# MartinErhardt/RoaringRegex

Measured on AMD Instinct MI355X. Metric: GB/s input scanned (whole job), 256-state regex, higher is better.
Workload: dtype u32

## Files before the change

### roaringregex_amd/csrc/corpus.cpp

```cpp
#include <algorithm>
#include <cstring>

#include "handles.hpp"

using namespace rrx;

namespace {
constexpr int kMailSlots = 64, kMailWords = 8;
struct MailPage { uint64_t *host = nullptr, *dev = nullptr; std::vector<int> free_slots; };
std::mutex g_mail_mu;
std::map<int, MailPage> g_mail;
}
int mailbox_acquire(int device, Mailbox *out) {
    std::lock_guard<std::mutex> lock(g_mail_mu);
    MailPage &pg = g_mail[device];
    if (!pg.host) {
        PinnedAlloc h;
        void *d = nullptr;
        hipError_t e = h.alloc(kMailSlots * kMailWords * sizeof(uint64_t), hipHostMallocMapped);
        if (e == hipSuccess) e = hipHostGetDevicePointer(&d, h.p, 0);
        if (e != hipSuccess) return hip_fail(e, "hipHostMalloc(mailbox)");
        pg.host = static_cast<uint64_t *>(h.release()); pg.dev = static_cast<uint64_t *>(d);
        for (int i = kMailSlots - 1; i >= 0; i--) pg.free_slots.push_back(i);
    }
    if (pg.free_slots.empty()) return fail(RRX_ERR_HIP, "more than 64 synchronous calls in flight on one device");
    out->slot = pg.free_slots.back(); pg.free_slots.pop_back();
    out->device = device;
    out->host = pg.host + (size_t)out->slot * kMailWords;
    out->dev = pg.dev + (size_t)out->slot * kMailWords;
    return RRX_OK;
}
void mailbox_release(const Mailbox &m) {
    if (m.slot < 0) return;
    std::lock_guard<std::mutex> lock(g_mail_mu);
    g_mail[m.device].free_slots.push_back(m.slot);
}

static constexpr uint32_t kSampleGroups = 8, kSampleBytes = 256;
static constexpr size_t kSampleMinCorpus = (size_t)64 << 20;

extern "C" {

int rrx_corpus_create(int device, const void *d_bytes, size_t nbytes, void *stream, rrx_corpus **out) {
    return rrx_corpus_create_ex(device, d_bytes, nbytes, 0, stream, out);
}

int rrx_corpus_create_ex(int device, const void *d_bytes, size_t nbytes, uint32_t stripe_bytes, void *stream, rrx_corpus **out) {
    if (!out || (nbytes && !d_bytes)) return fail(RRX_ERR_ARG, "null argument");
    if (stripe_bytes && (stripe_bytes < dev::kMinStripe || stripe_bytes > dev::kMaxStripe || (stripe_bytes & (stripe_bytes - 1))))
        return fail(RRX_ERR_ARG, "stripe must be a power of two in [512, 16384]");
    if (reinterpret_cast<uintptr_t>(d_bytes) & 15) return fail(RRX_ERR_ARG, "corpus base must be 16-byte aligned");
    *out = nullptr;
    HIP_TRY(hipSetDevice(device));
    std::unique_ptr<rrx_corpus> c(new rrx_corpus());
    c->device = device;
    c->d_bytes = static_cast<const uint8_t *>(d_bytes);
    c->nbytes = nbytes;
    c->stripe = stripe_bytes ? stripe_bytes : dev::pick_stripe(nbytes);
    constexpr size_t kSample = (size_t)4 << 20;
    if (!stripe_bytes && nbytes >= 16 * kSample) {
        rrx_corpus *sample = nullptr;
        if (rrx_corpus_create_ex(device, d_bytes, kSample, dev::pick_stripe(kSample), stream, &sample) == RRX_OK && sample) {
            if (sample->nlines) c->stripe = dev::stripe_for_lines(nbytes, kSample / sample->nlines);
            rrx_corpus_free(sample);
        }
    }
    c->nstripes = (nbytes + c->stripe - 1) / c->stripe;
    hipError_t e = c->d_counts.alloc(device, (c->nstripes + 3) * sizeof(uint32_t));
    if (e == hipSuccess) e = c->d_base.alloc(device, (c->nstripes + 1 + dev::scan_scratch_words(c->nstripes)) * sizeof(uint64_t));
    if (e != hipSuccess) return hip_fail(e, "hipMalloc(line index)");
    uint32_t *d_flags = c->d_counts + c->nstripes;
    e = hipMemsetAsync(d_flags, 0, 3 * sizeof(uint32_t), (hipStream_t)stream);
    if (e != hipSuccess) return hip_fail(e, "hipMemsetAsync(flags)");
    int rc = dev::count_newlines_per_stripe(c->d_bytes, nbytes, c->stripe, c->d_counts, c->nstripes, d_flags, stream);
    if (!rc) rc = dev::scan_counts(c->d_counts, c->d_base, c->d_base + c->nstripes + 1, c->nstripes, stream);
    if (!rc && c->nstripes) rc = dev::own_words_check(c->d_base, c->nstripes, c->d_bytes + nbytes - 1, d_flags + 1, stream);
    if (rc) return hip_fail((hipError_t)rc, "line index launch");
    MailboxGuard mail;
    if (int mrc = mailbox_acquire(device, &mail.m)) return mrc;
    if (nbytes >= kSampleMinCorpus && c->nstripes >= 64 * kSampleGroups &&
        c->h_sample.alloc((size_t)kSampleGroups * 32 * kSampleBytes) == hipSuccess) {
        c->sample_lanes = kSampleGroups * 32;
        for (uint32_t g = 0; g < kSampleGroups; g++) {
            const size_t first_stripe = (size_t)g * (c->nstripes / kSampleGroups);
            if (hipMemcpy2DAsync(c->h_sample + (size_t)g * 32 * kSampleBytes, kSampleBytes, c->d_bytes + first_stripe * c->stripe, c->stripe,
                                 kSampleBytes, 32, hipMemcpyDeviceToHost, (hipStream_t)stream) != hipSuccess) {
                (void)hipGetLastError();
                (void)hipStreamSynchronize((hipStream_t)stream);
                c->h_sample.reset(); c->sample_lanes = 0;
                break;
            }
        }
    }
    mail.stream = (hipStream_t)stream; mail.queued = true;
    rc = dev::mail_results(c->d_base + c->nstripes, d_flags, nbytes ? c->d_bytes + nbytes - 1 : nullptr, mail.m.dev, stream, d_flags + 1);
    if (rc) return hip_fail((hipError_t)rc, "line index launch");
    e = hipStreamSynchronize((hipStream_t)stream);
    if (e != hipSuccess) return hip_fail(e, "line index readback");
    mail.drained = true;
    const uint64_t total = mail.m.host[0];
    const uint32_t flags = (uint32_t)mail.m.host[1];
    const uint8_t last = nbytes ? (uint8_t)mail.m.host[2] : (uint8_t)'\n';
    c->has_high = (flags & 1u) != 0;
    c->own_words = c->nstripes && mail.m.host[3] == 0;
    c->own_span = (uint32_t)mail.m.host[4];
    c->nlines = (size_t)total + ((nbytes && last != '\n') ? 1 : 0);
    if (!stripe_bytes && c->nlines) {
        const uint32_t want = dev::stripe_for_lines(nbytes, nbytes / c->nlines);
        if (want != c->stripe) {
            c.reset();
            return rrx_corpus_create_ex(device, d_bytes, nbytes, want, stream, out);
        }
    }
    *out = c.release();
    return RRX_OK;
}
size_t rrx_corpus_num_lines(const rrx_corpus *c) { return c->nlines; }
size_t rrx_corpus_num_bytes(const rrx_corpus *c) { return c->nbytes; }
uint32_t rrx_corpus_stripe_bytes(const rrx_corpus *c) { return c->stripe; }
int rrx_corpus_one_launch(const rrx_corpus *c, uint32_t *span_words) {
    if (span_words) *span_words = c->own_words ? c->own_span : 0;
    return c->own_words ? 1 : 0;
}
void rrx_corpus_free(rrx_corpus *c) { delete c; }

size_t rrx_corpus_bitmap_words(const rrx_corpus *c) { return (c->nlines + 31) / 32; }

static int match_corpus_sampled(const rrx_regex *re, const rrx_corpus *c, const DeviceTables *t, uint32_t *d_accept_bits, void *stream) {
    dev::Dfa2Device d2;
    int rc = re->sampled_tables(c->device, &d2);
    if (rc) return rc;
    hipStream_t st = (hipStream_t)stream;
    const size_t words = rrx_corpus_bitmap_words(c);
    const size_t wide_bytes = (2 * words * sizeof(uint32_t) + 15) & ~(size_t)15, esc_bytes = (words * sizeof(uint32_t) + 15) & ~(size_t)15;
    const size_t cap = std::max<size_t>(words / 2, 1024);
    std::lock_guard<std::mutex> lock(re->onepass_mu);
    void *buf = nullptr;
    rc = re->onepass_for(c->device, wide_bytes + esc_bytes + cap * sizeof(uint64_t), &buf, st);
    if (rc) return rc;
    uint32_t *wide = static_cast<uint32_t *>(buf);
    uint32_t *escaped = reinterpret_cast<uint32_t *>(static_cast<uint8_t *>(buf) + wide_bytes);
    uint64_t *list = reinterpret_cast<uint64_t *>(static_cast<uint8_t *>(buf) + wide_bytes + esc_bytes);
    DeviceAlloc &count = re->sampled_dev.escapes[c->device];
    if (!count.p) HIP_TRY(count.alloc(c->device, 16));
    unsigned long long *total = static_cast<unsigned long long *>(count.p);
    constexpr uint32_t kSlots = kSampledRelearns + 1;
    PinnedArray<unsigned long long> &all_seen = re->sampled_dev.seen;
    if (!all_seen && all_seen.alloc(kSlots * sizeof(unsigned long long)) == hipSuccess)
        for (uint32_t k = 0; k < kSlots; k++) all_seen[k] = 0;
    unsigned long long *const seen = all_seen ? all_seen + re->sampled.seen_slot() : nullptr;
    if (seen) re->sampled.judge(seen[0]);
    hipError_t he = hipMemsetAsync(wide, 0, wide_bytes, st);
    if (he == hipSuccess) he = hipMemsetAsync(total, 0, 16, st);
    int e = he != hipSuccess ? (int)he : dev::match_stripes_dfa2_two_bit(d2, c->d_bytes, c->nbytes, c->stripe, c->d_base, c->nstripes, wide, stream);
    if (!e) e = dev::split_two_bit(wide, c->nlines, d_accept_bits, escaped, total, list, cap, stream);
    if (!e) e = dev::recheck_escaped_nfa(t->nfa, c->d_bytes, c->nbytes, c->stripe, c->d_base, c->nstripes, escaped, c->nlines, list, total, cap, d_accept_bits, stream);
    if (!e && seen) {
        if (hipMemcpyAsync(seen, total, sizeof(unsigned long long), hipMemcpyDeviceToHost, st) != hipSuccess) (void)hipGetLastError();
        re->sampled.queued(c->nlines);
    }
    const int rc2 = re->onepass_done(c->device, st);
    if (e) return hip_fail((hipError_t)e, "sampled-table launch");
    return rc2;
}

static unsigned long long *own_words_for(const rrx_corpus *c, const dev::Dfa2Device &d2, hipStream_t stream) {
    if (!c->own_words || c->own_span >= dev::dfa2_window_words(d2)) return nullptr;
    hipStreamCaptureStatus capture = hipStreamCaptureStatusNone;
    if (hipStreamIsCapturing(stream, &capture) != hipSuccess) { (void)hipGetLastError(); return nullptr; }
    if (capture != hipStreamCaptureStatusNone) return nullptr;
    std::lock_guard<std::mutex> lock(c->mu);
    auto it = c->slot_arrays.find(stream);
    if (it != c->slot_arrays.end()) return it->second;
    if (c->slot_arrays.size() >= rrx_corpus::kMaxSlotArrays) return nullptr;
    const size_t bytes = ((c->nstripes + dev::kThreads - 1) / dev::kThreads + 1) * sizeof(unsigned long long);
    DeviceArray<unsigned long long> slots;
    if (slots.alloc(c->device, bytes) != hipSuccess || hipMemsetAsync(slots, 0, bytes, stream) != hipSuccess) { (void)hipGetLastError(); return nullptr; }
    return c->slot_arrays.emplace(stream, std::move(slots)).first->second;
}
static uint32_t flush_mask_of(const rrx_regex *re, const rrx_corpus *c) {
    return re->opt_flush_slots.load() ? (uint32_t)re->opt_flush_slots.load() - 1u : dev::flush_mask_for(c->nbytes, c->nlines);
}
uint32_t rrx_match_flush_slots(const rrx_regex *re, const rrx_corpus *c, int *compiled_in) {
    const uint32_t mask = flush_mask_of(re, c);
    if (compiled_in) *compiled_in = dev::dfa2_flush_at_compile_time(mask) ? 1 : 0;
    return mask + 1;
}

static int launch_line_tables(const rrx_regex *re, const rrx_corpus *c, const LineTables &lt, const DeviceTables *t, bool stride2_over_high, uint32_t *bits,
                              void *stream) {
    const size_t words = rrx_corpus_bitmap_words(c);
    const bool stride2 = lt.has_dfa2 && (!c->has_high || stride2_over_high);
    dev::Dfa2Device d2;
    unsigned long long *slots = nullptr;
    if (stride2) { d2 = re->dfa2_device(t); slots = own_words_for(c, d2, (hipStream_t)stream); }
    if (!slots) HIP_TRY(hipMemsetAsync(bits, 0, words * sizeof(uint32_t), (hipStream_t)stream));
    if (!stride2) return launched(dev::match_stripes_dfa(t->line, c->has_high, c->d_bytes, c->nbytes, c->stripe, c->d_base, c->nstripes, bits, stream), "match_stripes launch");
    return launched(dev::match_stripes_dfa2(d2, c->has_high, c->d_bytes, c->nbytes, c->stripe, c->d_base, c->nstripes, bits, stream, flush_mask_of(re, c), slots, words),
                    "match_stripes launch");
}

int rrx_match_corpus(const rrx_regex *re, const rrx_corpus *c, uint32_t *d_accept_bits, void *stream) {
    if (!re || !c || (c->nlines && !d_accept_bits)) return fail(RRX_ERR_ARG, "null argument");
    if (!re->t2_order.decided() && c->h_sample && !c->has_high) (void)re->decide_t2_order(c->h_sample, c->sample_lanes, kSampleBytes, false);
    const DeviceTables *t;
    int rc = re->tables(c->device, &t);
    if (rc) return rc;
    HIP_TRY(hipSetDevice(c->device));
    if (!c->nlines) return RRX_OK;
    const bool sampled_on = re->opt_sampled_table.load() != 0;
    if (re->sampled.eligible() && sampled_on && !c->has_high) {
        const bool beside = re->opt_background_order.load() != 0;
        if (c->h_sample) (void)re->sampled.start_first(c->h_sample, c->sample_lanes, kSampleBytes, beside);
        if (c->h_sample && re->sampled.ready() && re->sampled.retired())
            re->sampled.start_relearn(c->h_sample, c->sample_lanes, kSampleBytes, beside);
        if (re->sampled.in_use(sampled_on)) return match_corpus_sampled(re, c, t, d_accept_bits, stream);
    }
    if (re->engine == RRX_ENGINE_DFA)
        return launch_line_tables(re, c, re->match, t, false, d_accept_bits, stream);
    HIP_TRY(hipMemsetAsync(d_accept_bits, 0, rrx_corpus_bitmap_words(c) * sizeof(uint32_t), (hipStream_t)stream));
    int e = 0;
    switch (re->engine) {
    case RRX_ENGINE_NFA_SPARSE: e = dev::match_stripes_sparse_nfa(t->block, c->d_bytes, c->nbytes, c->stripe, c->d_base, c->nstripes, d_accept_bits, stream); break;
    case RRX_ENGINE_NFA_BLOCK: e = dev::match_stripes_wave_nfa(t->block, c->d_bytes, c->nbytes, c->stripe, c->d_base, c->nstripes, d_accept_bits, stream); break;
    case RRX_ENGINE_NFA_WAVE: e = dev::match_stripes_group_nfa(t->group, c->d_bytes, c->nbytes, c->stripe, c->d_base, c->nstripes, d_accept_bits, stream); break;
    default: e = dev::match_stripes_nfa(t->nfa, c->d_bytes, c->nbytes, c->stripe, c->d_base, c->nstripes, d_accept_bits, stream);
    }
    return launched(e, "match_stripes launch");
}

int rrx_contains_corpus(const rrx_regex *re, const rrx_corpus *c, uint32_t *d_bits, void *stream) {
    if (!re || !c || (c->nlines && !d_bits)) return fail(RRX_ERR_ARG, "null argument");
    bool on_nfa = false, fill = false;
    const dev::NfaDevice *nfa = nullptr;
    int rc = re->contains_nfa_tables(c->device, &on_nfa, &nfa, &fill);
    if (rc) return rc;
    if (on_nfa) {
        HIP_TRY(hipSetDevice(c->device));
        if (!c->nlines) return RRX_OK;
        rc = fill_bitmap(d_bits, c->nlines, fill, stream);
        if (rc || !nfa) return rc;
        return launched(dev::contains_stripes_nfa(*nfa, c->d_bytes, c->nbytes, c->stripe, c->d_base, c->nstripes, d_bits, stream), "contains_stripes launch");
    }
    const DeviceTables *t;
    rc = re->contains_tables(c->device, &t);
    if (rc) return rc;
    HIP_TRY(hipSetDevice(c->device));
    if (!c->nlines) return RRX_OK;
    return launch_line_tables(re, c, re->contains_set.lt, t, true, d_bits, stream);
}
int rrx_bitmap_count(int device, const uint32_t *d_bits, size_t nlines, uint64_t *d_count, void *stream) {
    if (!d_count || (nlines && !d_bits)) return fail(RRX_ERR_ARG, "null argument");
    HIP_TRY(hipSetDevice(device));
    static_assert(sizeof(unsigned long long) == sizeof(uint64_t), "64-bit atomics");
    return launched(dev::bitmap_count(d_bits, nlines, reinterpret_cast<unsigned long long *>(d_count), stream), "bitmap_count launch");
}

int rrx_match_device(const rrx_regex *re, int device, const void *d_bytes, size_t nbytes, uint32_t *d_accept_bits, size_t cap_words,
                     size_t *nlines, void *stream) {
    if (!re || (nbytes && !d_bytes) || !nlines || (cap_words && !d_accept_bits)) return fail(RRX_ERR_ARG, "null argument");
    if (reinterpret_cast<uintptr_t>(d_bytes) & 15) return fail(RRX_ERR_ARG, "corpus base must be 16-byte aligned");
    *nlines = 0;
    HIP_TRY(hipSetDevice(device));
    if (!nbytes) return RRX_OK;
    hipStream_t st = static_cast<hipStream_t>(stream);
    const bool sampled = re->sampled.in_use(re->opt_sampled_table.load() != 0);
    if ((re->engine != RRX_ENGINE_DFA && re->engine != RRX_ENGINE_NFA) || sampled) {
        rrx_corpus *c = nullptr;
        int rc = rrx_corpus_create(device, d_bytes, nbytes, stream, &c);
        if (rc) return rc;
        *nlines = c->nlines;
        if (rrx_corpus_bitmap_words(c) > cap_words) rc = fail(RRX_ERR_ARG, "accept bitmap too small for the number of strings");
        if (!rc) rc = rrx_match_corpus(re, c, d_accept_bits, stream);
        const hipError_t e = hipStreamSynchronize(st);
        if (!rc && e != hipSuccess) rc = hip_fail(e, "match_device");
        rrx_corpus_free(c);
        return rc;
    }
    const DeviceTables *t;
    int rc = re->tables(device, &t);
    if (rc) return rc;
    const uint8_t *bytes = static_cast<const uint8_t *>(d_bytes);
    const uint32_t stripe = dev::pick_stripe(nbytes);
    const size_t nstripes = (nbytes + stripe - 1) / stripe;
    const size_t counts_bytes = ((nstripes + 2) * sizeof(uint32_t) + 15) & ~(size_t)15;
    const size_t base_bytes = (nstripes + 1 + dev::scan_scratch_words(nstripes)) * sizeof(uint64_t);
    const size_t slab_bytes = dev::onepass_slab_words(nstripes, stripe) * sizeof(uint32_t);
    std::lock_guard<std::mutex> lock(re->onepass_mu);
    void *buf = nullptr;
    rc = re->onepass_for(device, counts_bytes + base_bytes + slab_bytes, &buf, st);
    if (rc) return rc;
    uint32_t *d_counts = static_cast<uint32_t *>(buf);
    uint64_t *d_base = reinterpret_cast<uint64_t *>(static_cast<uint8_t *>(buf) + counts_bytes);
    uint32_t *d_slabs = reinterpret_cast<uint32_t *>(static_cast<uint8_t *>(buf) + counts_bytes + base_bytes);
    MailboxGuard mail;
    rc = mailbox_acquire(device, &mail.m);
    if (rc) return rc;
    if (cap_words) HIP_TRY(hipMemsetAsync(d_accept_bits, 0, cap_words * sizeof(uint32_t), st));
    int e = re->engine == RRX_ENGINE_NFA ? dev::match_onepass_nfa(t->nfa, bytes, nbytes, stripe, nstripes, d_counts, d_slabs, stream)
            : re->match.has_dfa2         ? dev::match_onepass_dfa2(re->dfa2_device(t), bytes, nbytes, stripe, nstripes, d_counts, d_slabs, stream)
                                         : dev::match_onepass_dfa(t->line, bytes, nbytes, stripe, nstripes, d_counts, d_slabs, stream);
    if (!e) e = dev::scan_counts(d_counts, d_base, d_base + nstripes + 1, nstripes, stream);
    if (!e) e = dev::compact_streams(d_counts, d_base, nstripes, stripe, d_slabs, d_accept_bits, cap_words, stream);
    mail.stream = st; mail.queued = true;
    if (!e) e = dev::mail_results(d_base + nstripes, nullptr, bytes + nbytes - 1, mail.m.dev, stream);
    if (e) return hip_fail((hipError_t)e, "one-pass launch");
    const hipError_t he = hipStreamSynchronize(st);
    if (he != hipSuccess) return hip_fail(he, "one-pass readback");
    mail.drained = true;
    *nlines = (size_t)mail.m.host[0] + ((uint8_t)mail.m.host[2] != '\n' ? 1 : 0);
    if ((*nlines + 31) / 32 > cap_words) return fail(RRX_ERR_ARG, "accept bitmap too small for the number of strings");
    return RRX_OK;
}

int rrx_bitmap_to_bytes(int device, const uint32_t *d_bits, size_t nlines, uint8_t *d_accept, void *stream) {
    if (nlines && (!d_bits || !d_accept)) return fail(RRX_ERR_ARG, "null argument");
    if (reinterpret_cast<uintptr_t>(d_accept) & 15) return fail(RRX_ERR_ARG, "byte buffer must be 16-byte aligned");
    HIP_TRY(hipSetDevice(device));
    return launched(dev::expand_bits(d_bits, nlines, d_accept, stream), "expand_bits launch");
}

static int match_host_chunk(const rrx_regex *re, int device, uint8_t *d_text, size_t len, hipStream_t st, uint32_t *d_bits,
                            uint8_t *d_acc, uint8_t *accept, size_t cap, size_t line_off, size_t *nlines_out) {
    rrx_corpus *c = nullptr;
    int rc = rrx_corpus_create(device, d_text, len, st, &c);
    if (rc) return rc;
    const size_t n = c->nlines;
    rc = rrx_match_corpus(re, c, d_bits, st);
    if (!rc) rc = rrx_bitmap_to_bytes(device, d_bits, n, d_acc, st);
    if (!rc && line_off < cap) {
        const size_t take = n < cap - line_off ? n : cap - line_off;
        hipError_t e = hipMemcpyAsync(accept + line_off, d_acc, take, hipMemcpyDeviceToHost, st);
        if (e != hipSuccess) rc = hip_fail(e, "accept readback");
    }
    hipError_t e = hipStreamSynchronize(st);
    if (!rc && e != hipSuccess) rc = hip_fail(e, "chunk sync");
    rrx_corpus_free(c);
    *nlines_out = n;
    return rc;
}

int rrx_match_host(const rrx_regex *re, int device, const void *bytes, size_t nbytes, uint8_t *accept, size_t cap, size_t *nlines) {
    if (!re || (nbytes && !bytes) || !nlines) return fail(RRX_ERR_ARG, "null argument");
    HIP_TRY(hipSetDevice(device));
    *nlines = 0;
    if (!nbytes) return RRX_OK;
    const uint8_t *host = static_cast<const uint8_t *>(bytes);
    const size_t kChunk = (size_t)256 << 20;
    const size_t buf_bytes = (nbytes < kChunk ? nbytes : kChunk) + 64;
    const size_t max_lines = buf_bytes;
    struct Lane {
        DeviceArray<uint8_t> text, acc;
        DeviceArray<uint32_t> bits;
        hipStream_t st = nullptr;
        ~Lane() { if (st) { (void)hipStreamSynchronize(st); (void)hipStreamDestroy(st); } }
    } lane[2];
    const int nbuf = nbytes > kChunk ? 2 : 1;
    int rc = RRX_OK;
    hipError_t e = hipSuccess;
    for (int i = 0; i < nbuf && e == hipSuccess; i++) {
        e = lane[i].text.alloc(device, buf_bytes);
        if (e == hipSuccess) e = lane[i].acc.alloc(device, max_lines + 64);
        if (e == hipSuccess) e = lane[i].bits.alloc(device, (max_lines / 32 + 4) * sizeof(uint32_t));
        if (e == hipSuccess) e = hipStreamCreate(&lane[i].st);
    }
    if (e != hipSuccess) rc = hip_fail(e, "pipeline buffers");

    std::vector<size_t> cuts{0};
    while (!rc && cuts.back() < nbytes) {
        size_t lo = cuts.back(), hi = lo + kChunk < nbytes ? lo + kChunk : nbytes;
        if (hi < nbytes) {
            size_t q = hi;
            while (q > lo && host[q - 1] != '\n') q--;
            if (q == lo) { rc = fail(RRX_ERR_UNSUPPORTED, "a single line longer than 256 MiB: use rrx_corpus_create on a device buffer"); break; }
            hi = q;
        }
        cuts.push_back(hi);
    }
    const size_t nchunks = cuts.size() - 1;
    size_t line_off = 0;
    if (!rc) {
        e = hipMemcpyAsync(lane[0].text, host, cuts[1] - cuts[0], hipMemcpyHostToDevice, lane[0].st);
        if (e != hipSuccess) rc = hip_fail(e, "chunk upload");
    }
    for (size_t i = 0; i < nchunks && !rc; i++) {
        const int cur = (int)(i & 1) % nbuf, nxt = (int)((i + 1) & 1) % nbuf;
        if (i + 1 < nchunks) {
            e = hipMemcpyAsync(lane[nxt].text, host + cuts[i + 1], cuts[i + 2] - cuts[i + 1], hipMemcpyHostToDevice, lane[nxt].st);
            if (e != hipSuccess) { rc = hip_fail(e, "chunk upload"); break; }
        }
        size_t n = 0;
        rc = match_host_chunk(re, device, lane[cur].text, cuts[i + 1] - cuts[i], lane[cur].st, lane[cur].bits, lane[cur].acc, accept, cap, line_off, &n);
        line_off += n;
    }
    for (int i = 0; i < nbuf; i++) if (lane[i].st) (void)hipStreamSynchronize(lane[i].st);
    *nlines = line_off;
    return rc;
}

}
```

### roaringregex_amd/csrc/device.hpp

```cpp
#pragma once
#include <cstddef>
#include <cstdint>

namespace rrx {
namespace dev {

#ifndef RRX_THREADS
#define RRX_THREADS 1024
#endif
constexpr int kThreads = RRX_THREADS;
constexpr uint32_t kMinStripe = 512, kMaxStripe = 16384, kMinAutoStripe = 2048;
constexpr size_t kTargetLanes = (size_t)1 << 21;
inline uint32_t pick_stripe(size_t nbytes) {
    uint32_t s = kMinStripe;
    while (s < kMinAutoStripe && nbytes / s > ((size_t)1 << 18)) s *= 2;
    while (s < kMaxStripe && nbytes / s > kTargetLanes) s *= 2;
    return s;
}
inline uint32_t stripe_for_lines(size_t nbytes, size_t avg_line) {
    uint32_t want = pick_stripe(nbytes);
    while (want < kMaxStripe && avg_line * 16 > want && nbytes / (2 * (size_t)want) >= ((size_t)1 << 18)) want *= 2;
    while (want > 1024 && (avg_line + 1) * 128 < want) want /= 2;
    return want;
}
constexpr int kRound = 128;
constexpr int kMaxNfaWords = 16;
constexpr uint32_t kWideColumns = 129;
constexpr uint32_t kWideMaxStates = 127;
constexpr uint32_t kClassedMaxEntries = 16384;

struct NfaMasks {
    uint32_t init[kMaxNfaWords], fin[kMaxNfaWords], chain[kMaxNfaWords], self[kMaxNfaWords], excm[kMaxNfaWords];
    uint32_t cgrp[kMaxNfaWords], ctgt[kMaxNfaWords];
};

struct NfaDevice {
    uint32_t W = 0, nbits = 0, any_exc = 0, any_carry = 0, any_self = 0;
    NfaMasks masks;
    const uint32_t *B = nullptr;
    const uint32_t *X = nullptr;
};

constexpr uint32_t kGroupMaxBits = 8192;
struct GroupNfaDevice {
    uint32_t G = 0, K = 0, nbits = 0, n_exc = 0, ncls = 0;
    uint32_t exc_mode = 0;
    uint32_t self_slots = 0;
    uint32_t b_slots = 0;
    uint32_t exc_slots = 0;
    const uint32_t *masks = nullptr;
    const uint32_t *Bcls = nullptr;
    const uint8_t *cls = nullptr;
    const uint16_t *xidx = nullptr;
    const uint32_t *X = nullptr;
};
inline bool group_geometry(uint32_t nbits, uint32_t *G, uint32_t *K) {
    static const uint32_t forms[][2] = {{8, 3}, {8, 4}, {16, 3}, {16, 4}, {32, 3}, {32, 4}, {32, 5}, {32, 8}};
    for (const auto &f : forms)
        if (nbits <= f[0] * f[1] * 32u) { *G = f[0]; *K = f[1]; return true; }
    return false;
}

constexpr uint32_t kBlockMaxBits = 65536;
struct WaveNfaDevice {
    uint32_t WL = 0, nbits = 0;
    uint32_t self_words = 0, exc_words = 0;
    const uint32_t *masks = nullptr;
    const uint32_t *Bbyte = nullptr;
    const uint32_t *xoff = nullptr;
    const uint32_t *xtgt = nullptr;
    uint32_t ncls = 0;
    const uint32_t *Bcls = nullptr;
    const uint8_t *cls = nullptr;
};

struct DfaDevice {
    uint32_t nstates = 0, ncls = 0, start = 0;
    const uint8_t *cls = nullptr;
    const uint16_t *next = nullptr;
    const uint8_t *acc = nullptr;
};

constexpr size_t kPlainDfaLdsBudget = 64 * 1024;

struct LineDfaDevice {
    uint32_t nrows = 0;
    uint32_t stride = 0;
    uint32_t start_off = 0;
    uint32_t wide = 0;
    uint32_t rep_log2 = 0;
    uint32_t in_global = 0;
    const uint32_t *table = nullptr;
    const uint8_t *cls = nullptr;
};

struct Dfa2Device {
    uint32_t nrows = 0, stride = 0, start_off = 0, rep_log2 = 0;
    const uint16_t *P = nullptr;
    const uint32_t *T2 = nullptr;
    const uint8_t *P8 = nullptr;
};
constexpr uint32_t kDfa2PStride = 130;
constexpr uint32_t kDfa2PBytes = 128 * kDfa2PStride * 2;
constexpr uint32_t kDfa2P8Stride = 136;
constexpr uint32_t kDfa2P8Bytes = 128 * kDfa2P8Stride;
constexpr uint32_t kDfa2PItemsBytes = (129 * kDfa2PStride * 2 + 15) & ~15u;
constexpr uint32_t kDfa2RegionBytes = 46 * 1024;
constexpr uint32_t kDfa2MaxTable = kDfa2RegionBytes - 4 * 1024;
constexpr uint32_t kDfa2TableBudget = 30 * 1024;


int match_stripes_dfa(const LineDfaDevice &p, bool clamp_high, const uint8_t *bytes, size_t nbytes, uint32_t stripe,
                      const uint64_t *stripe_base, size_t nstripes, uint32_t *accept_bits, void *stream);
uint32_t flush_mask_for(size_t nbytes, size_t nlines);
int match_stripes_dfa2(const Dfa2Device &p, bool clean, const uint8_t *bytes, size_t nbytes, uint32_t stripe, const uint64_t *stripe_base,
                       size_t nstripes, uint32_t *accept, void *stream, uint32_t flush_mask = 31u, unsigned long long *slots = nullptr,
                       size_t nwords = 0);
uint32_t dfa2_window_words(const Dfa2Device &p);
bool dfa2_flush_at_compile_time(uint32_t flush_mask);
int match_stripes_dfa2_two_bit(const Dfa2Device &p, const uint8_t *bytes, size_t nbytes, uint32_t stripe, const uint64_t *stripe_base,
                               size_t nstripes, uint32_t *wide_bits, void *stream);
int split_two_bit(const uint32_t *wide, size_t nlines, uint32_t *accept_bits, uint32_t *escaped_bits, unsigned long long *escaped_total, uint64_t *list,
                  size_t cap, void *stream);

size_t onepass_slab_words(size_t nstripes, uint32_t stripe);
int match_onepass_dfa2(const Dfa2Device &p, const uint8_t *bytes, size_t nbytes, uint32_t stripe, size_t nstripes, uint32_t *counts,
                       uint32_t *slabs, void *stream);
int match_onepass_dfa(const LineDfaDevice &p, const uint8_t *bytes, size_t nbytes, uint32_t stripe, size_t nstripes, uint32_t *counts,
                      uint32_t *slabs, void *stream);
int compact_streams(const uint32_t *counts, const uint64_t *stripe_base, size_t nstripes, uint32_t stripe, const uint32_t *slabs,
                    uint32_t *accept_bits, size_t cap_words, void *stream);
int match_extents_dfa(const DfaDevice &p, const uint8_t *bytes, const uint64_t *off, size_t nitems, uint32_t trim,
                      uint8_t *accept, void *stream, const uint32_t *only_if = nullptr);

int count_newlines_per_stripe(const uint8_t *bytes, size_t nbytes, uint32_t stripe, uint32_t *counts, size_t nstripes, uint32_t *flags, void *stream);
int scan_counts(const uint32_t *counts, uint64_t *base, uint64_t *chunk_sums, size_t n, void *stream);
size_t scan_scratch_words(size_t n);
int expand_bits(const uint32_t *bits, size_t nlines, uint8_t *out, void *stream);
int bitmap_count(const uint32_t *bits, size_t nlines, unsigned long long *count, void *stream);
int mail_results(const uint64_t *total, const uint32_t *flags, const uint8_t *last_byte, uint64_t *mail, void *stream, const uint32_t *own = nullptr);
int own_words_check(const uint64_t *stripe_base, size_t nstripes, const uint8_t *last_byte, uint32_t *own, void *stream);
int build_line_offsets(const uint8_t *bytes, size_t nbytes, uint32_t stripe, const uint64_t *stripe_base, size_t nstripes,
                       uint64_t *line_off, void *stream);
int empty_matches(const uint64_t *line_off, size_t nlines, uint32_t *count, const uint64_t *first, uint32_t *match_start, uint32_t *match_end,
                  void *stream, size_t cap = ~(size_t)0);

constexpr uint32_t kItemColumns = 131, kItemEndColumn = 129;
size_t items_index_bytes(size_t nbytes, size_t nitems);
size_t items_result_bytes(size_t nitems);
int items_index_build(size_t nbytes, const uint64_t *off, size_t nitems, uint32_t trim, void *index, uint32_t **flag, void *stream,
                      const uint8_t *resolve_base = nullptr, size_t min_bytes = 0);
struct ItemVerdicts {
    uint8_t *bytes = nullptr;
    uint32_t *bits = nullptr;
    ItemVerdicts(uint8_t *b) : bytes(b) {}
    ItemVerdicts(uint32_t *w) : bits(w) {}
};
int items_match2(const Dfa2Device &p, const uint8_t *bytes, size_t nbytes, size_t nitems, const void *index, void *result, ItemVerdicts out, void *stream,
                 const uint64_t *resolve_off = nullptr, const uint32_t *skip_if = nullptr);
int items_match(const LineDfaDevice &p, const uint8_t *bytes, size_t nbytes, size_t nitems, uint32_t trim, const void *index, void *result,
                ItemVerdicts out, void *stream, const uint64_t *resolve_off = nullptr, const uint32_t *skip_if = nullptr);

int contains_extents_dfa(const DfaDevice &p, bool in_global, uint32_t found, const uint8_t *bytes, const uint64_t *off, size_t nitems, uint32_t trim,
                         uint32_t *bits, void *stream, const uint32_t *only_if = nullptr);
int copy_result_bits(const uint32_t *result, size_t nitems, uint32_t *bits, void *stream);

struct MultiDevice {
    uint32_t nstates = 0, ncls = 0, start = 0, first_hit = 0, full = 0;
    const uint8_t *cls = nullptr;
    const uint16_t *next = nullptr;
    const uint32_t *mask = nullptr;
};
inline size_t multi_lds_bytes(uint32_t nstates, uint32_t ncls) {
    return (((size_t)nstates * ncls * 2 + 15) & ~(size_t)15) + 256 + (((size_t)nstates * 4 + 15) & ~(size_t)15);
}
int multi_contains_extents(const MultiDevice &p, bool in_global, bool first, const uint8_t *bytes, const uint64_t *off, size_t nitems, uint32_t trim,
                           uint32_t *out, void *stream);
int multi_counts(const uint32_t *mask, size_t nitems, unsigned long long *counts, void *stream);
int multi_plane(const uint32_t *mask, size_t nitems, uint32_t pattern, uint32_t *bits, void *stream);

int multi_contains_corpus(const MultiDevice &p, bool in_global, bool first, const uint8_t *bytes, size_t nbytes, uint32_t stripe, const uint64_t *stripe_base,
                          size_t nstripes, uint32_t *out, void *stream);

struct SearchItemsDevice {
    DfaDevice fwd, rev;
};
int search_extents_dfa(const SearchItemsDevice &p, bool in_global, const uint8_t *bytes, const uint64_t *off, size_t nitems, uint32_t trim,
                       uint32_t *match_start, uint32_t *match_end, void *stream);

int search_all_extents_dfa(const SearchItemsDevice &p, bool in_global, const uint8_t *bytes, const uint64_t *off, size_t nitems, uint32_t trim,
                           uint32_t *count, const uint64_t *first, uint32_t *match_start, uint32_t *match_end, size_t cap, void *stream);
int empty_item_matches(const uint64_t *off, size_t nitems, uint32_t trim, uint32_t *count, const uint64_t *first, uint32_t *match_start,
                       uint32_t *match_end, size_t cap, void *stream);

struct SearchLongestDevice {
    DfaDevice starts, anchored;
};
int search_longest_extents_dfa(const SearchLongestDevice &p, bool in_global, bool nullable, const uint8_t *bytes, const uint64_t *off, size_t nitems,
                               uint32_t trim, uint32_t *match_start, uint32_t *match_end, void *stream);

int search_longest_corpus_dfa(const SearchLongestDevice &p, bool in_global, bool nullable, const uint8_t *bytes, size_t nbytes, uint32_t stripe,
                              const uint64_t *stripe_base, size_t nstripes, uint32_t *match_start, uint32_t *match_end, void *stream);

size_t search_all_longest_marks_words(size_t extent_bytes, size_t nitems);
int search_all_longest_extents_dfa(const SearchLongestDevice &p, bool in_global, bool nullable, const uint8_t *bytes, const uint64_t *off, size_t nitems,
                                   uint32_t trim, uint32_t *marks, size_t marks_words, uint32_t *count, const uint64_t *first, uint32_t *match_start,
                                   uint32_t *match_end, size_t cap, void *stream);

struct GroupDevice {
    DfaDevice a, rev_bc, b, rev_c;
};
int longest_split_dfa(const DfaDevice &rev, const DfaDevice &fwd, bool in_global, const uint8_t *bytes, const uint64_t *off, size_t nitems, uint32_t trim,
                      const uint32_t *lo, const uint32_t *hi, uint32_t *marks, size_t marks_words, uint32_t *out, uint32_t *on_none, void *stream);

int longest_split_list_dfa(const DfaDevice &rev, const DfaDevice &fwd, bool in_global, const uint8_t *bytes, const uint64_t *off, size_t nitems,
                           uint32_t trim, const uint64_t *first, const uint32_t *lo, const uint32_t *hi, uint32_t *marks, size_t marks_words, uint32_t *out,
                           uint32_t *on_none, void *stream);
int slot_range_copy(const uint64_t *first, size_t nitems, const uint32_t *src_a, uint32_t *dst_a, const uint32_t *src_b, uint32_t *dst_b, void *stream);

constexpr size_t kReplaceMaxBlocks = 512;
int replace_sizes(const uint64_t *off, size_t nitems, uint32_t trim, const uint64_t *first, const uint32_t *match_start, const uint32_t *match_end,
                  uint32_t rep_len, uint32_t *len, uint32_t *pos, uint32_t *too_long, void *stream);
int replace_fill(const uint8_t *bytes, const uint64_t *off, size_t nitems, uint32_t trim, const uint64_t *first, const uint32_t *match_end,
                 const uint32_t *pos, const uint8_t *rep, uint32_t rep_len, const uint64_t *out_off, uint8_t *out, void *stream);

constexpr uint32_t kTemplateMaxSegments = 32;
struct TemplateDevice {
    const uint32_t *segs = nullptr;
    const uint8_t *lits = nullptr;
    uint32_t nseg = 0;
};
int replace_template_sizes(const TemplateDevice &tpl, const uint64_t *off, size_t nitems, uint32_t trim, const uint64_t *first, const uint32_t *match_start,
                           const uint32_t *match_end, const uint32_t *ref_start, const uint32_t *ref_end, uint64_t plane_stride, uint32_t *len, uint32_t *pos,
                           uint32_t *too_long, void *stream);
int replace_template_fill(const TemplateDevice &tpl, const uint8_t *bytes, const uint64_t *off, size_t nitems, uint32_t trim, const uint64_t *first,
                          const uint32_t *match_start, const uint32_t *match_end, const uint32_t *pos, const uint32_t *ref_start, const uint32_t *ref_end,
                          uint64_t plane_stride, const uint64_t *out_off, uint8_t *out, void *stream);

constexpr uint32_t kPiecesChunk = 4096;
constexpr size_t kPiecesMaxBlocks = kReplaceMaxBlocks;
int pieces_sizes(const uint64_t *off, size_t nitems, uint32_t trim, const uint64_t *first, const uint32_t *match_start, const uint32_t *match_end,
                 bool gaps, uint64_t *list_off, uint32_t *piece_len, uint64_t *piece_src, uint32_t *too_long, void *stream);
int pieces_fill(const uint8_t *bytes, const uint64_t *piece_src, const uint64_t *piece_off, size_t npieces, uint8_t *out, void *stream);

constexpr uint32_t kLongMaxStates = 254;
constexpr uint32_t kLongGroup = 128;
inline uint32_t long_chunk(size_t nbytes) {
    uint32_t chunk = 256;
    while (((nbytes + chunk - 1) / chunk) > (chunk < 1024 ? 1024u : 65536u)) chunk <<= 1;
    return chunk;
}
size_t long_scratch_bytes(uint32_t nstates, size_t nbytes, uint32_t *chunk);
int match_long_dfa(const DfaDevice &p, const uint8_t *bytes, size_t nbytes, uint32_t chunk, void *scratch, uint8_t *accept,
                   void *stream);

struct LongRunResult {
    uint64_t extreme;
    uint32_t exit_state, pad;
};
size_t long_run_scratch_bytes(uint32_t nstates, size_t nbytes);
int long_run_dfa(const DfaDevice &p, bool backward, bool row0_dead, const uint8_t *bytes, size_t nbytes, const uint32_t *start_state, void *scratch,
                 LongRunResult *out, void *stream);
int long_set_word(uint32_t *word, uint32_t value, void *stream);

constexpr uint32_t kSearchP8Stride = 132, kSearchP8Bytes = 128 * kSearchP8Stride;
constexpr uint32_t kSearchP16Stride = 130, kSearchP16Bytes = 128 * kSearchP16Stride * 2;
struct SearchChunkDevice {
    uint32_t nrows = 0, ncols2 = 0, row_bytes = 0, base_row = 0, in_global = 0;
    uint32_t start_row = 0, skip_row = 0;
    uint32_t nr = 0, ncls = 0, start_r = 0;
    const uint8_t *P8 = nullptr;
    const uint16_t *P16 = nullptr;
    const uint16_t *T2 = nullptr, *T2_all = nullptr;
    const uint32_t *G2 = nullptr, *G2_all = nullptr;
    const uint16_t *rev = nullptr;
    const uint8_t *cls = nullptr;
};
constexpr size_t kSearchChunkLdsBudget = 160 * 1024;
size_t search_chunk_bytes();
size_t search_chunks_lds_bytes(const SearchChunkDevice &p);
int search_chunks(const SearchChunkDevice &p, bool clean, const uint8_t *bytes, size_t nbytes, const uint64_t *chunk_base, size_t nchunks, size_t nlines,
                  uint32_t *match_start, uint32_t *match_end, void *stream);
int search_chunks_count(const SearchChunkDevice &p, bool clean, const uint8_t *bytes, size_t nbytes, const uint64_t *chunk_base, size_t nchunks,
                        uint32_t *count, void *stream);
int search_chunks_fill(const SearchChunkDevice &p, bool clean, const uint8_t *bytes, size_t nbytes, const uint64_t *chunk_base, size_t nchunks,
                       const uint64_t *first, uint32_t *match_start, uint32_t *match_end, void *stream);
size_t search_all_scratch_bytes(size_t nchunks);
int search_chunks_all(const SearchChunkDevice &p, bool clean, const uint8_t *bytes, size_t nbytes, const uint64_t *chunk_base, size_t nchunks, size_t nlines,
                      uint64_t *first, uint32_t *match_start, uint32_t *match_end, size_t cap, void *scratch, void *stream);

int match_stripes_nfa(const NfaDevice &p, const uint8_t *bytes, size_t nbytes, uint32_t stripe, const uint64_t *stripe_base,
                      size_t nstripes, uint32_t *accept_bits, void *stream);
int match_onepass_nfa(const NfaDevice &p, const uint8_t *bytes, size_t nbytes, uint32_t stripe, size_t nstripes, uint32_t *counts,
                      uint32_t *slabs, void *stream);
int recheck_escaped_nfa(const NfaDevice &p, const uint8_t *bytes, size_t nbytes, uint32_t stripe, const uint64_t *stripe_base, size_t nstripes,
                        const uint32_t *escaped_bits, size_t nlines, const uint64_t *list, const unsigned long long *escaped_total, size_t cap,
                        uint32_t *accept_bits, void *stream);
int match_extents_nfa(const NfaDevice &p, const uint8_t *bytes, const uint64_t *off, size_t nitems, uint32_t trim,
                      uint8_t *accept, void *stream);
int contains_stripes_nfa(const NfaDevice &p, const uint8_t *bytes, size_t nbytes, uint32_t stripe, const uint64_t *stripe_base,
                         size_t nstripes, uint32_t *bits, void *stream);
int contains_extents_nfa(const NfaDevice &p, const uint8_t *bytes, const uint64_t *off, size_t nitems, uint32_t trim, uint32_t *bits,
                         void *stream);
size_t long_nfa_scratch_bytes(const NfaDevice &p, size_t nbytes, uint32_t *chunk, uint32_t *nchunks);
int match_long_nfa(const NfaDevice &p, const uint8_t *bytes, size_t nbytes, uint32_t chunk, uint32_t nchunks, void *scratch, uint8_t *accept,
                   void *stream);

int match_stripes_group_nfa(const GroupNfaDevice &p, const uint8_t *bytes, size_t nbytes, uint32_t stripe, const uint64_t *stripe_base,
                            size_t nstripes, uint32_t *accept_bits, void *stream);
int match_extents_group_nfa(const GroupNfaDevice &p, const uint8_t *bytes, const uint64_t *off, size_t nitems, uint32_t trim,
                            uint8_t *accept, void *stream);

uint32_t wave_words_per_lane(uint32_t words);
uint32_t sparse_rows(uint32_t words);
int match_stripes_sparse_nfa(const WaveNfaDevice &p, const uint8_t *bytes, size_t nbytes, uint32_t stripe, const uint64_t *stripe_base,
                             size_t nstripes, uint32_t *accept_bits, void *stream);
int match_extents_sparse_nfa(const WaveNfaDevice &p, const uint8_t *bytes, const uint64_t *off, size_t nitems, uint32_t trim,
                             uint8_t *accept, void *stream);
int match_stripes_wave_nfa(const WaveNfaDevice &p, const uint8_t *bytes, size_t nbytes, uint32_t stripe, const uint64_t *stripe_base,
                           size_t nstripes, uint32_t *accept_bits, void *stream);
int match_extents_wave_nfa(const WaveNfaDevice &p, const uint8_t *bytes, const uint64_t *off, size_t nitems, uint32_t trim,
                           uint8_t *accept, void *stream);

}
}
```

### roaringregex_amd/csrc/kernels_common.hpp

```cpp
#pragma once
#include <hip/hip_runtime.h>

#include <atomic>
#include <type_traits>

#include "device.hpp"

namespace rrx {
namespace dev {
namespace {

constexpr uint32_t kEndsOnNewline = 0x80000000u;
constexpr uint64_t kFreshStripe = 1ull << 63;
__device__ __forceinline__ uint64_t line_of(uint64_t base) { return base & ~kFreshStripe; }

__device__ __forceinline__ uint4 load_text(const uint4 *p) { return *p; }

__device__ __forceinline__ uint32_t newline_flags(uint32_t w) {
    const uint32_t t = w ^ 0x0a0a0a0au;
    return ~(((t & 0x7f7f7f7fu) + 0x7f7f7f7fu) | t) & 0x80808080u;
}

template <int kBatch = 4>
__device__ __forceinline__ void copy_table_to_lds(void *dst_lds, const void *src, uint32_t nbytes, uint32_t add = 0) {
    uint4 *d = static_cast<uint4 *>(dst_lds);
    const uint4 *s = static_cast<const uint4 *>(src);
    const uint32_t nvec = nbytes / 16;
    for (uint32_t base = threadIdx.x; base < nvec; base += kBatch * blockDim.x) {
        uint4 v[kBatch];
#pragma unroll
        for (int k = 0; k < kBatch; k++) {
            const uint32_t i = base + k * blockDim.x;
            if (i < nvec) v[k] = s[i];
        }
#pragma unroll
        for (int k = 0; k < kBatch; k++) {
            const uint32_t i = base + k * blockDim.x;
            if (i < nvec) d[i] = make_uint4(v[k].x + add, v[k].y + add, v[k].z + add, v[k].w + add);
        }
    }
    const uint32_t tail = nvec * 4 + threadIdx.x;
    if (tail < nbytes / 4) static_cast<uint32_t *>(dst_lds)[tail] = static_cast<const uint32_t *>(src)[tail] + add;
}

template <int N>
struct TextRound {
    uint4 head;
    TextRound<N - 1> rest;
    __device__ __forceinline__ void load(const uint4 *p) { head = load_text(p); rest.load(p + 1); }
    template <class F> __device__ __forceinline__ void for_each_slot(F &&f) const { f(head); rest.for_each_slot(f); }
    template <class F> __device__ __forceinline__ void for_each_slot_down(F &&f) const { rest.for_each_slot_down(f); f(head); }
    template <class F> __device__ __forceinline__ void for_each_slot_mut(F &&f) { f(head); rest.for_each_slot_mut(f); }
};
template <>
struct TextRound<0> {
    __device__ __forceinline__ void load(const uint4 *) {}
    template <class F> __device__ __forceinline__ void for_each_slot(F &&) const {}
    template <class F> __device__ __forceinline__ void for_each_slot_down(F &&) const {}
    template <class F> __device__ __forceinline__ void for_each_slot_mut(F &&) {}
};

constexpr uint32_t kStageWords = 4096;
template <bool STAGED>
struct ResultsT {
    uint32_t bits = 1;
    uint32_t outw = 0;
    uint32_t fill;
    uint32_t seen = 0;
    typename std::conditional<STAGED, uint32_t, uint64_t>::type word;
    bool drop_first;
    uint32_t drop_mask = 1u;
    bool writer = true;
    uint32_t *__restrict__ out;
    uint32_t *stage = nullptr;
    uint32_t stage_words = kStageWords;

    __device__ __forceinline__ void begin(uint64_t first_line, bool drop, uint32_t *bitmap) {
        word = first_line >> 5; fill = (uint32_t)first_line & 31u; drop_first = drop; out = bitmap;
    }
    __device__ __forceinline__ void begin_staged(uint64_t first_line, uint64_t window_word, bool drop, uint32_t *bitmap, uint32_t *lds) {
        word = (decltype(word))((first_line >> 5) - window_word); fill = (uint32_t)first_line & 31u; drop_first = drop;
        out = bitmap + window_word; stage = lds;
    }
    __device__ __forceinline__ void emit() {
        if (!outw || !writer) return;
        if (STAGED && word < stage_words) atomicOr(&stage[(uint32_t)word], outw);
        else atomicOr(&out[word], outw);
    }
    __device__ __forceinline__ void push(uint32_t nl, uint32_t acc) { bits = (bits << nl) | acc; }
    __device__ __forceinline__ void flush() {
        const int n = 31 - __clz((int)bits);
        if (n > 0) {
            uint32_t rev = __brev(bits & ((1u << n) - 1u)) >> (32 - n);
            if (drop_first) { rev &= ~drop_mask; drop_first = false; }
            outw |= rev << fill;
            uint32_t nf = fill + (uint32_t)n;
            if (nf >= 32u) {
                emit();
                word++;
                outw = rev >> (32u - fill);
                nf -= 32u;
            }
            fill = nf;
            seen += (uint32_t)n;
            bits = 1;
        }
    }
    __device__ __forceinline__ void finish() {
        flush();
        emit();
        outw = 0;
    }
};
typedef ResultsT<false> Results;

struct LocalResults {
    uint32_t bits = 1, outw = 0, fill = 0, seen = 0, k = 0;
    uint32_t *__restrict__ dst;
    uint32_t row;
    __device__ __forceinline__ void begin(uint32_t *slab_lane, uint32_t row_stripes) { dst = slab_lane; row = row_stripes; }
    __device__ __forceinline__ void push(uint32_t nl, uint32_t acc) { bits = (bits << nl) | acc; }
    __device__ __forceinline__ void flush() {
        const int n = 31 - __clz((int)bits);
        if (n > 0) {
            const uint32_t rev = __brev(bits & ((1u << n) - 1u)) >> (32 - n);
            outw |= rev << fill;
            uint32_t nf = fill + (uint32_t)n;
            if (nf >= 32u) {
                dst[(size_t)k * row] = outw;
                k++;
                outw = fill ? rev >> (32u - fill) : 0u;
                nf -= 32u;
            }
            fill = nf;
            seen += (uint32_t)n;
            bits = 1;
        }
    }
    __device__ __forceinline__ void finish() {
        flush();
        if (fill) dst[(size_t)k * row] = outw;
    }
};
constexpr uint32_t kCountMask = 0x3fffffffu;
constexpr uint32_t kExtraResult = 0x40000000u;
__host__ __device__ inline size_t slab_words_per_lane(uint32_t stripe) { return stripe / 32 + 1; }

template <class Engine, class Program, bool ONEPASS = false>
__device__ __forceinline__ void match_stripes_body(const Program &prog, const uint8_t *__restrict__ bytes, size_t nbytes,
                                                   uint32_t stripe, const uint64_t *__restrict__ stripe_base,
                                                   uint32_t *__restrict__ accept_bits, uint32_t stage_off, uint32_t stage_words,
                                                   uint32_t *__restrict__ counts = nullptr, uint32_t *__restrict__ slabs = nullptr) {
    extern __shared__ __attribute__((aligned(16))) uint8_t smem[];
    constexpr bool kWindow = Engine::kStaged && !ONEPASS;
    uint32_t *stage = reinterpret_cast<uint32_t *>(smem + stage_off);
    Engine eng;
    eng.load(prog, smem);
    if (kWindow)
        for (uint32_t i = threadIdx.x; i < stage_words; i += kThreads) stage[i] = 0;
    __syncthreads();

    const size_t g0 = (size_t)blockIdx.x * kThreads;
    uint64_t window_word = 0;
    if (!ONEPASS) window_word = line_of(stripe_base[g0]) >> 5;
    const size_t g = g0 + threadIdx.x;
    const size_t start = g * (size_t)stripe;
    if (start < nbytes) {
    const size_t stripe_end = start + stripe;
    const size_t my_end = stripe_end < nbytes ? stripe_end : nbytes;
    bool fresh = true;
    typename std::conditional<ONEPASS, LocalResults, ResultsT<Engine::kStaged>>::type res;
    if constexpr (ONEPASS) {
        res.begin(slabs + g, gridDim.x * kThreads);
    } else {
        const uint64_t my_base = stripe_base[g];
        fresh = (my_base & kFreshStripe) != 0;
        if constexpr (Engine::kStaged) { res.begin_staged(line_of(my_base), window_word, !fresh, accept_bits, stage); res.stage_words = stage_words; }
        else res.begin(line_of(my_base), !fresh, accept_bits);
    }
    typename Engine::State st = fresh ? eng.fresh() : eng.skipping();

    size_t pos = start;
    const uint4 *src = reinterpret_cast<const uint4 *>(bytes + start);
    constexpr int kSlots = Engine::kRoundBytes / 16;
    const int rounds = (int)((my_end - start) / Engine::kRoundBytes);
    TextRound<kSlots> buf;
    if (rounds > 0) buf.load(src);
    for (int r = 0; r < rounds; r++) {
        buf.for_each_slot([&](const uint4 &v) {
            const uint32_t w[4] = {v.x, v.y, v.z, v.w};
#pragma unroll
            for (int q = 0; q < 4; q++) eng.consume_word(st, w[q], res.bits);
            if (res.bits >> 15) res.flush();
        });
        if ((r & (512 / Engine::kRoundBytes - 1)) == 512 / Engine::kRoundBytes - 1) res.flush();
        if (r + 1 < rounds) buf.load(src + (size_t)(r + 1) * kSlots);
    }
    pos += (size_t)rounds * Engine::kRoundBytes;

    for (; pos < my_end; pos++) {
        uint32_t nl, acc;
        eng.step(st, bytes[pos], nl, acc);
        res.push(nl, acc);
        if (res.bits >> 30) res.flush();
    }
    res.flush();
    const uint32_t newlines = res.seen;

    if (ONEPASS && res.seen == 0) fresh = g == 0 || bytes[start - 1] == '\n';
    const bool started = fresh || res.seen > 0;
    bool followed = false;
    if (started && bytes[my_end - 1] != '\n') {
        uint32_t nl = 0, acc = 0;
        while (pos + 16 <= nbytes && !nl) {
            const uint4 v = *reinterpret_cast<const uint4 *>(bytes + pos);
            const uint32_t w[4] = {v.x, v.y, v.z, v.w};
#pragma unroll
            for (int k = 0; k < 16; k++)
                if (!nl) eng.step(st, (w[k >> 2] >> (8 * (k & 3))) & 0xffu, nl, acc);
            pos += 16;
        }
        for (; pos < nbytes && !nl; pos++) eng.step(st, bytes[pos], nl, acc);
        if (!nl) eng.step(st, '\n', nl, acc);
        res.push(nl, acc);
        followed = true;
    }
    res.finish();
    if (ONEPASS) counts[g] = newlines | (followed ? kExtraResult : 0u) | (bytes[my_end - 1] == '\n' ? kEndsOnNewline : 0u);
    }
    if (kWindow) {
        __syncthreads();
        for (uint32_t i = threadIdx.x; i < stage_words; i += kThreads) {
            const uint32_t v = stage[i];
            if (v) atomicOr(&accept_bits[window_word + i], v);
        }
    }
}

template <class Engine, class Program>
__global__ __launch_bounds__(kThreads) void match_stripes_kernel(Program prog, const uint8_t *__restrict__ bytes, size_t nbytes,
                                                                  uint32_t stripe, const uint64_t *__restrict__ stripe_base,
                                                                  uint32_t *__restrict__ accept_bits, uint32_t stage_off,
                                                                  uint32_t stage_words) {
    match_stripes_body<Engine, Program>(prog, bytes, nbytes, stripe, stripe_base, accept_bits, stage_off, stage_words);
}
template <class Engine, class Program>
__global__ __launch_bounds__(kThreads) __attribute__((amdgpu_waves_per_eu(8, 8)))
void match_stripes_kernel_8waves(Program prog, const uint8_t *__restrict__ bytes, size_t nbytes, uint32_t stripe,
                                 const uint64_t *__restrict__ stripe_base, uint32_t *__restrict__ accept_bits, uint32_t stage_off,
                                 uint32_t stage_words) {
    match_stripes_body<Engine, Program>(prog, bytes, nbytes, stripe, stripe_base, accept_bits, stage_off, stage_words);
}
template <class Engine, class Program>
__global__ __launch_bounds__(kThreads) void match_stripes_onepass_kernel(Program prog, const uint8_t *__restrict__ bytes, size_t nbytes, uint32_t stripe,
                                                                          uint32_t *__restrict__ counts, uint32_t *__restrict__ slabs) {
    match_stripes_body<Engine, Program, true>(prog, bytes, nbytes, stripe, nullptr, nullptr, 0, 0, counts, slabs);
}
constexpr int kMaxDevices = 64;
struct LdsAttr { std::atomic<int> bytes[kMaxDevices]; std::atomic<int> at_zero_ok{0}; };
inline hipError_t ensure_dynamic_lds(LdsAttr &slots, const void *kernel, size_t bytes, bool at_zero = false) {
    if (at_zero && !slots.at_zero_ok.load(std::memory_order_acquire)) {
        hipFuncAttributes fa;
        hipError_t e = hipFuncGetAttributes(&fa, kernel);
        if (e != hipSuccess) return e;
        if (fa.sharedSizeBytes != 0) return hipErrorInvalidConfiguration;
        slots.at_zero_ok.store(1, std::memory_order_release);
    }
    int dev = 0;
    hipError_t e = hipGetDevice(&dev);
    if (e != hipSuccess) return e;
    if (dev < 0 || dev >= kMaxDevices) return hipFuncSetAttribute(kernel, hipFuncAttributeMaxDynamicSharedMemorySize, (int)bytes);
    if (slots.bytes[dev].load(std::memory_order_acquire) >= (int)bytes) return hipSuccess;
    e = hipFuncSetAttribute(kernel, hipFuncAttributeMaxDynamicSharedMemorySize, (int)bytes);
    if (e == hipSuccess) slots.bytes[dev].store((int)bytes, std::memory_order_release);
    return e;
}
template <class Engine, class = void> struct lds_at_zero : std::false_type {};
template <class Engine> struct lds_at_zero<Engine, std::enable_if_t<Engine::kLdsAtZero>> : std::true_type {};

template <class Engine, class Program>
int launch_stripes(const Program &p, size_t table_bytes, const uint8_t *bytes, size_t nbytes, uint32_t stripe,
                   const uint64_t *stripe_base, size_t nstripes, uint32_t *accept, void *stream) {
    if (!nstripes) return 0;
    void (*k)(Program, const uint8_t *, size_t, uint32_t, const uint64_t *, uint32_t *, uint32_t, uint32_t);
    if constexpr (Engine::kEightWaves) k = match_stripes_kernel_8waves<Engine, Program>;
    else k = match_stripes_kernel<Engine, Program>;
    const uint32_t stage_off = (uint32_t)((table_bytes + 15) & ~(size_t)15);
    const size_t half_cu = 80 * 1024;
    const uint32_t stage_words = stage_off + kStageWords * sizeof(uint32_t) >= half_cu ? kStageWords : (uint32_t)((half_cu - stage_off) / 4);
    const size_t lds = Engine::kStaged ? stage_off + (size_t)stage_words * sizeof(uint32_t) : table_bytes;
    static LdsAttr attr;
    hipError_t e = ensure_dynamic_lds(attr, reinterpret_cast<const void *>(k), lds, lds_at_zero<Engine>::value);
    if (e != hipSuccess) return (int)e;
    size_t blocks = (nstripes + kThreads - 1) / kThreads;
    hipLaunchKernelGGL(k, dim3((unsigned)blocks), dim3(kThreads), lds, (hipStream_t)stream, p, bytes, nbytes, stripe, stripe_base, accept, stage_off, stage_words);
    return (int)hipGetLastError();
}

template <class Engine, class Program>
int launch_onepass(const Program &p, size_t table_bytes, const uint8_t *bytes, size_t nbytes, uint32_t stripe, size_t nstripes, uint32_t *counts,
                   uint32_t *slabs, void *stream) {
    if (!nstripes) return 0;
    auto k = match_stripes_onepass_kernel<Engine, Program>;
    static LdsAttr attr;
    hipError_t e = ensure_dynamic_lds(attr, reinterpret_cast<const void *>(k), table_bytes, lds_at_zero<Engine>::value);
    if (e != hipSuccess) return (int)e;
    size_t blocks = (nstripes + kThreads - 1) / kThreads;
    hipLaunchKernelGGL(k, dim3((unsigned)blocks), dim3(kThreads), table_bytes, (hipStream_t)stream, p, bytes, nbytes, stripe, counts, slabs);
    return (int)hipGetLastError();
}

}
}
}
```

### roaringregex_amd/csrc/kernels_coop.hip

```cpp
#include "kernels_common.hpp"

namespace rrx {
namespace dev {
namespace {

template <int G, int K, int MODE, bool SLOT0>
struct GroupNfa {
    uint32_t fin[K], self[K], exc[K], x0[K];
    typedef const __attribute__((address_space(3))) uint32_t *lds_u32_ptr;
    typedef const __attribute__((address_space(3))) uint8_t *lds_u8_ptr;
    lds_u32_ptr rows;
    lds_u8_ptr cls;
    const uint16_t *__restrict__ xidx;
    const uint32_t *__restrict__ X;
    uint32_t self_slots, b_slots, exc_slots;
    int lane, lig, gbase;
    uint64_t gmask;

    static size_t lds_bytes(const GroupNfaDevice &p) { return (size_t)p.ncls * G * K * 4 + 256; }
    __device__ void load(const GroupNfaDevice &p, uint8_t *lds) {
        uint32_t *r = reinterpret_cast<uint32_t *>(lds);
        const int n = (int)(p.ncls * G * K);
        for (int i = threadIdx.x; i < n; i += blockDim.x) r[i] = p.Bcls[i];
        uint8_t *c = lds + (size_t)n * 4;
        for (int i = threadIdx.x; i < 256; i += blockDim.x) c[i] = p.cls[i];
        lane = threadIdx.x & 63; lig = lane & (G - 1); gbase = lane - lig;
        rows = (lds_u32_ptr)(__attribute__((address_space(3))) uint8_t *)lds + K * lig;
        cls = (lds_u8_ptr)(__attribute__((address_space(3))) uint8_t *)c;
        gmask = (G == 64 ? ~0ull : ((1ull << G) - 1ull)) << gbase;
        self_slots = p.self_slots; b_slots = p.b_slots; exc_slots = p.exc_slots;
#pragma unroll
        for (int k = 0; k < K; k++) {
            fin[k] = p.masks[(0 * G + lig) * K + k]; self[k] = p.masks[(1 * G + lig) * K + k]; exc[k] = p.masks[(2 * G + lig) * K + k];
            x0[k] = 0;
        }
        xidx = p.xidx; X = p.X;
        if (MODE == 2) {
#pragma unroll
            for (int k = 0; k < K; k++) x0[k] = X[((size_t)xidx[0] * G + lig) * K + k];
        }
    }
    struct State { uint32_t s[K]; bool dead; };
    __device__ __forceinline__ bool accepting(const State &st) const {
        uint32_t any = 0;
#pragma unroll
        for (int k = 0; k < K; k++) any |= st.s[k] & fin[k];
        return !st.dead && (__ballot(any != 0) & gmask) != 0;
    }
    __device__ __forceinline__ void line_start(State &st) const {
#pragma unroll
        for (int k = 0; k < K; k++) st.s[k] = 0;
        if (lig == 0) st.s[0] = 1u;
        st.dead = false;
    }
    __device__ __forceinline__ void kill(State &st) const {
#pragma unroll
        for (int k = 0; k < K; k++) st.s[k] = 0;
    }
    struct Row { uint32_t b[SLOT0 ? 1 : K]; bool kills; };
    __device__ __forceinline__ uint32_t class_of(uint32_t c) const { return cls[c]; }
    __device__ __forceinline__ Row fetch(uint32_t cl) const {
        lds_u32_ptr row = rows + cl * (uint32_t)(G * K);
        Row r;
#pragma unroll
        for (int k = 0; k < (SLOT0 ? 1 : K); k++) r.b[k] = row[k];
        r.kills = cl == 0u;
        return r;
    }
    __device__ __forceinline__ void advance(State &st, uint32_t c, bool first = false) const { step(st, fetch(class_of(c)), first); }
    __device__ __forceinline__ void step(State &st, const Row &r, bool first = false) const {
        if (SLOT0) st.dead = st.dead || r.kills;
        uint32_t below;
        if (G == 16) below = __builtin_amdgcn_update_dpp(0u, st.s[K - 1], 0x111 , 0xf, 0xf, true);
        else if (G == 8) {
            below = __builtin_amdgcn_update_dpp(0u, st.s[K - 1], 0x111 , 0xf, 0xf, true);
            if (lig == 0) below = 0u;
        } else {
            below = __builtin_amdgcn_update_dpp(0u, st.s[K - 1], 0x138 , 0xf, 0xf, true);
            if (lig == 0) below = 0u;
        }
        uint32_t t[K];
        t[0] = __builtin_amdgcn_alignbit(st.s[0], below, 31);
#pragma unroll
        for (int k = 1; k < K; k++) t[k] = __builtin_amdgcn_alignbit(st.s[k], st.s[k - 1], 31);
#pragma unroll
        for (int k = 0; k < (SLOT0 ? 1 : K); k++) t[k] |= st.s[k] & self[k];
        if (MODE == 2) {
            if (first) {
#pragma unroll
                for (int k = 0; k < K; k++) t[k] |= x0[k];
            }
        } else if (exc_slots) {
            uint32_t mine_pos = 0xffffffffu;
            uint32_t e[K];
#pragma unroll
            for (int k = K - 1; k >= 0; k--) {
                e[k] = st.s[k] & exc[k];
                if (e[k]) mine_pos = (uint32_t)((lig * K + k) * 32) + (uint32_t)__ffs((int)e[k]) - 1u;
            }
            uint64_t live = __ballot(mine_pos != 0xffffffffu);
            while (live) {
                const uint64_t mine = live & gmask;
                const int src = mine ? __ffsll((long long)mine) - 1 : lane;
                const uint32_t pos = __shfl(mine_pos, src, 64);
                if (mine) {
                    if (lane == src) {
                        const uint32_t slot = (pos >> 5) - (uint32_t)(lig * K), bit = pos & 31u;
                        mine_pos = 0xffffffffu;
#pragma unroll
                        for (int k = K - 1; k >= 0; k--) {
                            if ((uint32_t)k == slot) e[k] &= ~(1u << bit);
                            if (e[k]) mine_pos = (uint32_t)((lig * K + k) * 32) + (uint32_t)__ffs((int)e[k]) - 1u;
                        }
                    }
                    const uint32_t *xr = X + ((size_t)xidx[pos] * G + lig) * K;
#pragma unroll
                    for (int k = 0; k < K; k++) t[k] |= xr[k];
                }
                live = __ballot(mine_pos != 0xffffffffu);
            }
        }
#pragma unroll
        for (int k = 0; k < K; k++) st.s[k] = (SLOT0 && k > 0) ? t[k] : (t[k] & r.b[SLOT0 ? 0 : k]);
    }
};

template <int G, int K, int MODE, bool SLOT0>
__global__ __launch_bounds__(256) void match_stripes_group_kernel(GroupNfaDevice prog, const uint8_t *__restrict__ bytes, size_t nbytes,
                                                                   uint32_t stripe1, uint32_t span, const uint64_t *__restrict__ stripe_base,
                                                                   uint32_t *__restrict__ accept_bits) {
    extern __shared__ __attribute__((aligned(16))) uint8_t smem[];
    typedef GroupNfa<G, K, MODE, SLOT0> Eng;
    Eng eng;
    eng.load(prog, smem);
    __syncthreads();
    const size_t g = ((size_t)blockIdx.x * 256 + threadIdx.x) / G;
    const size_t stripe = (size_t)stripe1 * span;
    const size_t start = g * stripe;
    if (start >= nbytes) return;
    const size_t stripe_end = start + stripe;
    const size_t my_end = stripe_end < nbytes ? stripe_end : nbytes;
    const uint64_t my_base = stripe_base[g * span];
    const bool fresh = (my_base & kFreshStripe) != 0;
    typename Eng::State st;
    eng.line_start(st);
    bool first = fresh;
    if (!fresh) eng.kill(st);
    Results res;
    res.begin(line_of(my_base), !fresh, accept_bits);
    res.writer = eng.lig == 0;

    auto one_row = [&](uint32_t c, const typename Eng::Row &row) {
        const bool isnl = c == '\n';
        typename Eng::State a = st;
        eng.step(a, row, first);
        first = false;
        if (__ballot(isnl)) {
            const bool ok = eng.accepting(st);
            if (isnl) { res.push(1, ok ? 1u : 0u); if (res.bits >> 30) res.flush(); eng.line_start(a); first = true; }
        }
        st = a;
    };
    auto one = [&](uint32_t c) { one_row(c, eng.fetch(eng.class_of(c))); };
    size_t pos = start;
    for (; pos + 16 <= my_end; pos += 16) {
        const uint4 v = *reinterpret_cast<const uint4 *>(bytes + pos);
        const uint32_t w[4] = {v.x, v.y, v.z, v.w};
        uint32_t nl = 0;
#pragma unroll
        for (int q = 0; q < 4; q++) { const uint32_t x = w[q] ^ 0x0a0a0a0au; nl |= ~(((x & 0x7f7f7f7fu) + 0x7f7f7f7fu) | x | 0x7f7f7f7fu); }
        if (!__ballot(nl != 0 || (MODE == 2 && first))) {
            uint32_t cl[16];
#pragma unroll
            for (int k = 0; k < 16; k++) cl[k] = eng.class_of((w[k >> 2] >> (8 * (k & 3))) & 0xffu);
#pragma unroll
            for (int q = 0; q < 4; q++) {
                const typename Eng::Row r0 = eng.fetch(cl[4 * q]), r1 = eng.fetch(cl[4 * q + 1]), r2 = eng.fetch(cl[4 * q + 2]), r3 = eng.fetch(cl[4 * q + 3]);
                eng.step(st, r0); eng.step(st, r1); eng.step(st, r2); eng.step(st, r3);
            }
        } else {
#pragma unroll 1
            for (int q = 0; q < 4; q++) {
                const uint32_t wq = q < 2 ? (q == 0 ? v.x : v.y) : (q == 2 ? v.z : v.w);
                const uint32_t c0 = wq & 0xffu, c1 = (wq >> 8) & 0xffu, c2 = (wq >> 16) & 0xffu, c3 = wq >> 24;
                const uint32_t l0 = eng.class_of(c0), l1 = eng.class_of(c1), l2 = eng.class_of(c2), l3 = eng.class_of(c3);
                const typename Eng::Row r0 = eng.fetch(l0), r1 = eng.fetch(l1), r2 = eng.fetch(l2), r3 = eng.fetch(l3);
                one_row(c0, r0); one_row(c1, r1); one_row(c2, r2); one_row(c3, r3);
            }
        }
    }
    for (; pos < my_end; pos++) one(bytes[pos]);
    res.flush();

    const bool started = fresh || res.seen > 0;
    if (started && bytes[my_end - 1] != '\n') {
        bool ended = false;
        while (!ended && !(pos & 15) && pos + 16 <= nbytes) {
            const uint4 v = *reinterpret_cast<const uint4 *>(bytes + pos);
#pragma unroll 1
            for (int k = 0; k < 16 && !ended; k++) {
                const uint32_t wk = k < 8 ? (k < 4 ? v.x : v.y) : (k < 12 ? v.z : v.w);
                const uint32_t c = (wk >> (8 * (k & 3))) & 0xffu;
                if (c == '\n') ended = true;
                else { eng.advance(st, c, first); first = false; }
            }
            pos += 16;
        }
        for (; pos < nbytes && !ended; pos++) {
            const uint32_t c = bytes[pos];
            if (c == '\n') ended = true;
            else { eng.advance(st, c, first); first = false; }
        }
        res.push(1, eng.accepting(st) ? 1u : 0u);
    }
    res.finish();
}

template <int G, int K, int MODE, bool SLOT0>
__global__ __launch_bounds__(256) void match_extents_group_kernel(GroupNfaDevice prog, const uint8_t *__restrict__ bytes,
                                                                   const uint64_t *__restrict__ off, size_t nitems, uint32_t trim,
                                                                   uint8_t *__restrict__ accept) {
    extern __shared__ __attribute__((aligned(16))) uint8_t smem[];
    typedef GroupNfa<G, K, MODE, SLOT0> Eng;
    Eng eng;
    eng.load(prog, smem);
    __syncthreads();
    const size_t i = ((size_t)blockIdx.x * 256 + threadIdx.x) / G;
    if (i >= nitems) return;
    size_t b = off[i], e = off[i + 1];
    e = e - b >= trim ? e - trim : b;
    typename Eng::State st;
    eng.line_start(st);
    for (size_t pos = b; pos < e; pos++) eng.advance(st, bytes[pos], pos == b);
    const bool ok = eng.accepting(st);
    if (eng.lig == 0) accept[i] = ok ? 1 : 0;
}

}

template <int G, int K, int MODE, bool SLOT0>
static int launch_group_stripes(const GroupNfaDevice &p, const uint8_t *bytes, size_t nbytes, uint32_t stripe, const uint64_t *stripe_base,
                                size_t nstripes, uint32_t *accept, void *stream) {
    const size_t lds = GroupNfa<G, K, MODE, SLOT0>::lds_bytes(p);
    if (lds > 128 * 1024) return (int)hipErrorInvalidValue;
    static LdsAttr attr;
    hipError_t e = ensure_dynamic_lds(attr, reinterpret_cast<const void *>(match_stripes_group_kernel<G, K, MODE, SLOT0>), lds);
    if (e != hipSuccess) return (int)e;
    const size_t resident_groups = (size_t)256 * 28 * (64 / G);
    uint32_t span = 1;
    while ((size_t)stripe * span * 2 <= 16384 && nstripes / (2 * (size_t)span) >= 2 * resident_groups) span *= 2;
    const size_t ngroups = (nstripes + span - 1) / span;
    const size_t per_block = 256 / G, blocks = (ngroups + per_block - 1) / per_block;
    hipLaunchKernelGGL((match_stripes_group_kernel<G, K, MODE, SLOT0>), dim3((unsigned)blocks), dim3(256), lds, (hipStream_t)stream, p, bytes, nbytes, stripe, span,
                       stripe_base, accept);
    return (int)hipGetLastError();
}
template <int G, int K, int MODE, bool SLOT0>
static int launch_group_extents(const GroupNfaDevice &p, const uint8_t *bytes, const uint64_t *off, size_t nitems, uint32_t trim, uint8_t *accept,
                                void *stream) {
    const size_t lds = GroupNfa<G, K, MODE, SLOT0>::lds_bytes(p);
    if (lds > 128 * 1024) return (int)hipErrorInvalidValue;
    static LdsAttr attr;
    hipError_t e = ensure_dynamic_lds(attr, reinterpret_cast<const void *>(match_extents_group_kernel<G, K, MODE, SLOT0>), lds);
    if (e != hipSuccess) return (int)e;
    const size_t per_block = 256 / G, blocks = (nitems + per_block - 1) / per_block;
    hipLaunchKernelGGL((match_extents_group_kernel<G, K, MODE, SLOT0>), dim3((unsigned)blocks), dim3(256), lds, (hipStream_t)stream, p, bytes, off, nitems, trim, accept);
    return (int)hipGetLastError();
}
#define RRX_GROUP_FORM(FN, GG, KK, ...)                                                                  \
    if (p.G == GG && p.K == KK)                                                                          \
        return p.exc_mode != 2 ? FN<GG, KK, 0, false>(__VA_ARGS__) : slot0 ? FN<GG, KK, 2, true>(__VA_ARGS__) : FN<GG, KK, 2, false>(__VA_ARGS__);
#define RRX_GROUP_DISPATCH(FN, ...)                                                                      \
    const bool slot0 = ((p.b_slots | p.self_slots) & ~1u) == 0u;                                         \
    RRX_GROUP_FORM(FN, 8, 3, __VA_ARGS__) RRX_GROUP_FORM(FN, 8, 4, __VA_ARGS__)                                             \
    RRX_GROUP_FORM(FN, 16, 3, __VA_ARGS__) RRX_GROUP_FORM(FN, 16, 4, __VA_ARGS__)                                           \
    RRX_GROUP_FORM(FN, 32, 3, __VA_ARGS__) RRX_GROUP_FORM(FN, 32, 4, __VA_ARGS__) RRX_GROUP_FORM(FN, 32, 5, __VA_ARGS__)    \
    RRX_GROUP_FORM(FN, 32, 8, __VA_ARGS__)                                                                                  \
    return (int)hipErrorInvalidValue;
int match_stripes_group_nfa(const GroupNfaDevice &p, const uint8_t *bytes, size_t nbytes, uint32_t stripe, const uint64_t *stripe_base,
                            size_t nstripes, uint32_t *accept, void *stream) {
    if (!nstripes) return 0;
    RRX_GROUP_DISPATCH(launch_group_stripes, p, bytes, nbytes, stripe, stripe_base, nstripes, accept, stream)
}
int match_extents_group_nfa(const GroupNfaDevice &p, const uint8_t *bytes, const uint64_t *off, size_t nitems, uint32_t trim, uint8_t *accept,
                            void *stream) {
    if (!nitems) return 0;
    RRX_GROUP_DISPATCH(launch_group_extents, p, bytes, off, nitems, trim, accept, stream)
}
#undef RRX_GROUP_DISPATCH
#undef RRX_GROUP_FORM
#define RRX_NFA_PARTS(name, ARGS_DECL, ARGS)                                                        \
    int name##_part0 ARGS_DECL; int name##_part1 ARGS_DECL; int name##_part2 ARGS_DECL; int name##_part3 ARGS_DECL; \
    int name ARGS_DECL { return p.W <= 2 ? name##_part0 ARGS : p.W <= 4 ? name##_part1 ARGS : p.W <= 8 ? name##_part2 ARGS : name##_part3 ARGS; }
RRX_NFA_PARTS(match_stripes_nfa,
              (const NfaDevice &p, const uint8_t *bytes, size_t nbytes, uint32_t stripe, const uint64_t *stripe_base, size_t nstripes, uint32_t *accept, void *stream),
              (p, bytes, nbytes, stripe, stripe_base, nstripes, accept, stream))
RRX_NFA_PARTS(match_onepass_nfa,
              (const NfaDevice &p, const uint8_t *bytes, size_t nbytes, uint32_t stripe, size_t nstripes, uint32_t *counts, uint32_t *slabs, void *stream),
              (p, bytes, nbytes, stripe, nstripes, counts, slabs, stream))
RRX_NFA_PARTS(match_extents_nfa,
              (const NfaDevice &p, const uint8_t *bytes, const uint64_t *off, size_t nitems, uint32_t trim, uint8_t *accept, void *stream),
              (p, bytes, off, nitems, trim, accept, stream))
RRX_NFA_PARTS(contains_stripes_nfa,
              (const NfaDevice &p, const uint8_t *bytes, size_t nbytes, uint32_t stripe, const uint64_t *stripe_base, size_t nstripes, uint32_t *bits, void *stream),
              (p, bytes, nbytes, stripe, stripe_base, nstripes, bits, stream))
RRX_NFA_PARTS(contains_extents_nfa,
              (const NfaDevice &p, const uint8_t *bytes, const uint64_t *off, size_t nitems, uint32_t trim, uint32_t *bits, void *stream),
              (p, bytes, off, nitems, trim, bits, stream))
RRX_NFA_PARTS(recheck_escaped_nfa,
              (const NfaDevice &p, const uint8_t *bytes, size_t nbytes, uint32_t stripe, const uint64_t *stripe_base, size_t nstripes, const uint32_t *escaped_bits,
               size_t nlines, const uint64_t *list, const unsigned long long *escaped_total, size_t cap, uint32_t *accept_bits, void *stream),
              (p, bytes, nbytes, stripe, stripe_base, nstripes, escaped_bits, nlines, list, escaped_total, cap, accept_bits, stream))
RRX_NFA_PARTS(match_long_nfa,
              (const NfaDevice &p, const uint8_t *bytes, size_t nbytes, uint32_t chunk, uint32_t nchunks, void *scratch, uint8_t *accept, void *stream),
              (p, bytes, nbytes, chunk, nchunks, scratch, accept, stream))
#undef RRX_NFA_PARTS
size_t long_nfa_scratch_bytes(const NfaDevice &p, size_t nbytes, uint32_t *chunk, uint32_t *nchunks) {
    uint32_t c = 1024;
    const size_t per_chunk = (size_t)p.nbits * p.W * 4;
    while ((nbytes + c - 1) / c > 65536 || ((nbytes + c - 1) / c) * per_chunk > ((size_t)256 << 20)) c <<= 1;
    *chunk = c;
    *nchunks = (uint32_t)((nbytes + c - 1) / c);
    return ((size_t)*nchunks + ((size_t)*nchunks + 1) / 2) * per_chunk;
}
}
}
```

### roaringregex_amd/csrc/kernels_index.hip

```cpp
#include "kernels_common.hpp"

namespace rrx {
namespace dev {
namespace {

__global__ void mail_results_kernel(const uint64_t *__restrict__ total, const uint32_t *__restrict__ flags, const uint8_t *__restrict__ last_byte,
                                    uint64_t *__restrict__ mail, const uint32_t *__restrict__ own) {
    if (threadIdx.x || blockIdx.x) return;
    mail[0] = line_of(*total);
    mail[1] = flags ? *flags : 0u;
    mail[2] = last_byte ? *last_byte : (uint64_t)'\n';
    mail[3] = own ? own[0] : 0u;
    mail[4] = own ? own[1] : 0u;
    __threadfence_system();
}

__global__ __launch_bounds__(256) void own_words_kernel(const uint64_t *__restrict__ stripe_base, size_t nstripes, size_t nworkgroups,
                                                        const uint8_t *__restrict__ last_byte, uint32_t *__restrict__ own) {
    const size_t b = (size_t)blockIdx.x * 256 + threadIdx.x;
    if (b >= nworkgroups) return;
    const uint64_t first = line_of(stripe_base[b * kThreads]) >> 5;
    uint64_t last;
    if (b + 1 < nworkgroups) {
        last = line_of(stripe_base[(b + 1) * kThreads]) >> 5;
        if (last <= first) { atomicOr(&own[0], 1u); return; }
    } else {
        const uint64_t nlines = line_of(stripe_base[nstripes]) + (*last_byte != '\n' ? 1u : 0u);
        last = (nlines - 1) >> 5;
    }
    const uint64_t span = last - first;
    atomicMax(&own[1], span < 0xffffffffull ? (uint32_t)span : 0xffffffffu);
}

__global__ __launch_bounds__(256) void count_newlines_kernel(const uint8_t *__restrict__ bytes, size_t nbytes, uint32_t stripe,
                                                              uint32_t *__restrict__ counts, size_t nstripes,
                                                              uint32_t *__restrict__ flags) {
    const size_t g = (size_t)blockIdx.x * 256 + threadIdx.x;
    if (g >= nstripes) return;
    const size_t start = g * (size_t)stripe;
    const size_t end = start + stripe < nbytes ? start + stripe : nbytes;
    const uint4 *src = reinterpret_cast<const uint4 *>(bytes + start);
    const int units = (int)((end - start) / 16);
    uint32_t cnt = 0, high = 0;
    int u = 0;
    for (; u + 4 <= units; u += 4) {
        uint4 v[4];
#pragma unroll
        for (int i = 0; i < 4; i++) v[i] = src[u + i];
#pragma unroll
        for (int i = 0; i < 4; i++) {
            const uint32_t w[4] = {v[i].x, v[i].y, v[i].z, v[i].w};
#pragma unroll
            for (int j = 0; j < 4; j++) {
                uint32_t x = w[j] ^ 0x0a0a0a0au;
                uint32_t z = ~(((x & 0x7f7f7f7fu) + 0x7f7f7f7fu) | x | 0x7f7f7f7fu);
                cnt += __popc(z);
                high |= w[j];
            }
        }
    }
    for (size_t p = start + (size_t)u * 16; p < end; p++) { cnt += bytes[p] == '\n'; high |= bytes[p]; }
    counts[g] = cnt | (bytes[end - 1] == '\n' ? kEndsOnNewline : 0u);
    if (high & 0x80808080u) atomicOr(flags, 1u);
}

__global__ __launch_bounds__(256) void count_newlines_wave_kernel(const uint8_t *__restrict__ bytes, size_t nbytes, uint32_t stripe,
                                                                   uint32_t *__restrict__ counts, size_t nstripes,
                                                                   uint32_t *__restrict__ flags) {
    const int lane = threadIdx.x & 63;
    const size_t nwaves = (size_t)gridDim.x * 4;
    uint32_t high = 0;
    for (size_t g = ((size_t)blockIdx.x * 256 + threadIdx.x) >> 6; g < nstripes; g += nwaves) {
        const size_t start = g * (size_t)stripe;
        const size_t end = start + stripe < nbytes ? start + stripe : nbytes;
        uint32_t cnt = 0, last = 0;
        if (end - start == stripe) {
            const uint4 *src = reinterpret_cast<const uint4 *>(bytes + start) + lane;
            const int n = (int)(stripe >> 10);
            for (int i = 0; i < n; i += 4) {
                uint4 v[4];
#pragma unroll
                for (int k = 0; k < 4; k++)
                    if (i + k < n) v[k] = src[(size_t)(i + k) * 64];
#pragma unroll
                for (int k = 0; k < 4; k++) {
                    if (i + k < n) {
                        const uint32_t w[4] = {v[k].x, v[k].y, v[k].z, v[k].w};
#pragma unroll
                        for (int j = 0; j < 4; j++) {
                            const uint32_t x = w[j] ^ 0x0a0a0a0au;
                            const uint32_t z = ~(((x & 0x7f7f7f7fu) + 0x7f7f7f7fu) | x | 0x7f7f7f7fu);
                            cnt += __popc(z);
                            high |= w[j];
                        }
                        last = v[k].w >> 24;
                    }
                }
            }
            last = __shfl(last, 63, 64);
        } else {
            for (size_t p = start + lane; p < end; p += 64) { const uint32_t b = bytes[p]; cnt += b == '\n'; high |= b; }
            last = bytes[end - 1];
        }
#pragma unroll
        for (int d = 32; d; d >>= 1) cnt += __shfl_xor(cnt, d, 64);
        if (lane == 0) counts[g] = cnt | (last == '\n' ? kEndsOnNewline : 0u);
    }
    if (__ballot((high & 0x80808080u) != 0) && lane == 0) atomicOr(flags, 1u);
}

__global__ __launch_bounds__(256) void expand_bits_kernel(const uint32_t *__restrict__ bits, size_t nlines, uint8_t *__restrict__ out) {
    const size_t w = (size_t)blockIdx.x * 256 + threadIdx.x;
    if (w * 32 >= nlines) return;
    const uint32_t v = bits[w];
    if (w * 32 + 32 <= nlines) {
        uint4 o[2];
        uint32_t *p = reinterpret_cast<uint32_t *>(o);
#pragma unroll
        for (int j = 0; j < 8; j++) {
            uint32_t n = (v >> (4 * j)) & 0xfu;
            p[j] = (n & 1u) | ((n & 2u) << 7) | ((n & 4u) << 14) | ((n & 8u) << 21);
        }
        uint4 *dst = reinterpret_cast<uint4 *>(out + w * 32);
        dst[0] = o[0]; dst[1] = o[1];
    } else {
        for (size_t i = w * 32; i < nlines; i++) out[i] = (uint8_t)((v >> (i & 31)) & 1u);
    }
}

constexpr int kScanChunk = 4096;
__global__ __launch_bounds__(256) void scan_chunk_sums_kernel(const uint32_t *__restrict__ counts, size_t n, uint64_t *__restrict__ sums) {
    __shared__ uint64_t part[4];
    const size_t lo = (size_t)blockIdx.x * kScanChunk;
    uint64_t s = 0;
    for (size_t i = lo + threadIdx.x; i < lo + kScanChunk && i < n; i += 256) s += counts[i] & kCountMask;
#pragma unroll
    for (int d = 32; d; d >>= 1) s += __shfl_down(s, d, 64);
    if ((threadIdx.x & 63) == 0) part[threadIdx.x >> 6] = s;
    __syncthreads();
    if (threadIdx.x == 0) sums[blockIdx.x] = part[0] + part[1] + part[2] + part[3];
}
template <int NW>
__device__ __forceinline__ uint64_t block_exclusive_scan(uint64_t v, uint64_t *wave_tot, uint64_t &total) {
    const int lane = threadIdx.x & 63, wave = threadIdx.x >> 6;
    uint64_t inc = v;
#pragma unroll
    for (int d = 1; d < 64; d <<= 1) {
        const uint64_t o = __shfl_up(inc, d, 64);
        if (lane >= d) inc += o;
    }
    if (lane == 63) wave_tot[wave] = inc;
    __syncthreads();
    uint64_t off = 0, tot = 0;
#pragma unroll
    for (int w = 0; w < NW; w++) {
        const uint64_t t = wave_tot[w];
        if (w < wave) off += t;
        tot += t;
    }
    total = tot;
    return off + inc - v;
}
__global__ __launch_bounds__(1024) void scan_sums_kernel(uint64_t *__restrict__ sums, size_t nchunks, uint64_t *__restrict__ total) {
    __shared__ uint64_t wave_tot[16];
    const size_t per = (nchunks + 1023) / 1024;
    const size_t lo = threadIdx.x * per < nchunks ? threadIdx.x * per : nchunks, hi = lo + per < nchunks ? lo + per : nchunks;
    uint64_t s = 0;
    for (size_t i = lo; i < hi; i++) s += sums[i];
    uint64_t all;
    uint64_t run = block_exclusive_scan<16>(s, wave_tot, all);
    if (threadIdx.x == 0) *total = all;
    for (size_t i = lo; i < hi; i++) { uint64_t v = sums[i]; sums[i] = run; run += v; }
}
__global__ __launch_bounds__(256) void scan_chunks_kernel(const uint32_t *__restrict__ counts, size_t n, const uint64_t *__restrict__ sums,
                                                           uint64_t *__restrict__ base) {
    __shared__ uint64_t wave_tot[4];
    constexpr int kPer = kScanChunk / 256;
    const size_t lo = (size_t)blockIdx.x * kScanChunk + (size_t)threadIdx.x * kPer;
    uint32_t c[kPer];
    uint32_t before = 0;
    if (lo + kPer <= n) {
        const uint4 *src = reinterpret_cast<const uint4 *>(counts + lo);
#pragma unroll
        for (int k = 0; k < kPer / 4; k++) { const uint4 v = src[k]; c[4 * k] = v.x; c[4 * k + 1] = v.y; c[4 * k + 2] = v.z; c[4 * k + 3] = v.w; }
    } else {
#pragma unroll
        for (int k = 0; k < kPer; k++) c[k] = lo + k < n ? counts[lo + k] : 0u;
    }
    if (lo && lo < n) before = counts[lo - 1];
    uint64_t s = 0;
#pragma unroll
    for (int k = 0; k < kPer; k++) s += c[k] & kCountMask;
    uint64_t all;
    uint64_t run = sums[blockIdx.x] + block_exclusive_scan<4>(s, wave_tot, all);
#pragma unroll
    for (int k = 0; k < kPer; k++) {
        if (lo + k < n) {
            const bool fresh = lo + k == 0 || ((k ? c[k - 1] : before) & kEndsOnNewline);
            base[lo + k] = run | (fresh ? kFreshStripe : 0);
        }
        run += c[k] & kCountMask;
    }
}

__global__ __launch_bounds__(256) void line_offsets_kernel(const uint8_t *__restrict__ bytes, size_t nbytes, uint32_t stripe,
                                                           const uint64_t *__restrict__ stripe_base, size_t nstripes,
                                                           uint64_t *__restrict__ line_off) {
    const size_t g = (size_t)blockIdx.x * blockDim.x + threadIdx.x;
    if (g >= nstripes) return;
    const size_t start = g * (size_t)stripe, end = start + stripe < nbytes ? start + stripe : nbytes;
    uint64_t line = line_of(stripe_base[g]);
    if (g == 0) line_off[0] = 0;
    size_t pos = start;
    for (; pos + 16 <= end; pos += 16) {
        const uint4 v = *reinterpret_cast<const uint4 *>(bytes + pos);
        const uint32_t w[4] = {v.x, v.y, v.z, v.w};
#pragma unroll
        for (int j = 0; j < 4; j++) {
            const uint32_t x = w[j] ^ 0x0a0a0a0au;
            uint32_t hit = (x - 0x01010101u) & ~x & 0x80808080u;
            while (hit) {
                const int k = (__ffs((int)hit) - 1) >> 3;
                if (((w[j] >> (8 * k)) & 0xffu) == '\n') line_off[++line] = pos + 4 * j + k + 1;
                hit &= hit - 1;
            }
        }
    }
    for (; pos < end; pos++)
        if (bytes[pos] == '\n') line_off[++line] = pos + 1;
}

template <bool FILL>
__global__ __launch_bounds__(256) void empty_matches_kernel(const uint64_t *__restrict__ line_off, size_t nlines, uint32_t *__restrict__ count,
                                                            const uint64_t *__restrict__ first, uint32_t *__restrict__ match_start,
                                                            uint32_t *__restrict__ match_end, uint64_t cap) {
    const size_t i = (size_t)blockIdx.x * blockDim.x + threadIdx.x;
    if (i >= nlines) return;
    const uint64_t len = line_off[i + 1] - 1 - line_off[i];
    if (!FILL) { count[i] = (uint32_t)(len + 1); return; }
    const uint64_t slot = first[i];
    for (uint64_t k = 0; k <= len && slot + k < cap; k++) { match_start[slot + k] = (uint32_t)k; match_end[slot + k] = (uint32_t)k; }
}

}

int count_newlines_per_stripe(const uint8_t *bytes, size_t nbytes, uint32_t stripe, uint32_t *counts, size_t nstripes, uint32_t *flags,
                              void *stream) {
    if (!nstripes) return 0;
    if (stripe % 1024 == 0 && stripe >= 4096) {
        size_t blocks = (nstripes + 3) / 4;
        if (blocks > 8192) blocks = 8192;
        hipLaunchKernelGGL(count_newlines_wave_kernel, dim3((unsigned)blocks), dim3(256), 0, (hipStream_t)stream, bytes, nbytes, stripe, counts, nstripes, flags);
        return (int)hipGetLastError();
    }
    size_t blocks = (nstripes + 255) / 256;
    hipLaunchKernelGGL(count_newlines_kernel, dim3((unsigned)blocks), dim3(256), 0, (hipStream_t)stream, bytes, nbytes, stripe, counts, nstripes, flags);
    return (int)hipGetLastError();
}
int expand_bits(const uint32_t *bits, size_t nlines, uint8_t *out, void *stream) {
    if (!nlines) return 0;
    size_t words = (nlines + 31) / 32, blocks = (words + 255) / 256;
    hipLaunchKernelGGL(expand_bits_kernel, dim3((unsigned)blocks), dim3(256), 0, (hipStream_t)stream, bits, nlines, out);
    return (int)hipGetLastError();
}
int scan_counts(const uint32_t *counts, uint64_t *base, uint64_t *chunk_sums, size_t n, void *stream) {
    const size_t nchunks = (n + kScanChunk - 1) / kScanChunk;
    hipStream_t st = (hipStream_t)stream;
    if (nchunks) hipLaunchKernelGGL(scan_chunk_sums_kernel, dim3((unsigned)nchunks), dim3(256), 0, st, counts, n, chunk_sums);
    hipLaunchKernelGGL(scan_sums_kernel, dim3(1), dim3(1024), 0, st, chunk_sums, nchunks, base + n);
    if (nchunks) hipLaunchKernelGGL(scan_chunks_kernel, dim3((unsigned)nchunks), dim3(256), 0, st, counts, n, chunk_sums, base);
    return (int)hipGetLastError();
}
size_t scan_scratch_words(size_t n) { return (n + kScanChunk - 1) / kScanChunk + 1; }
__global__ __launch_bounds__(256) void bitmap_count_kernel(const uint32_t *__restrict__ bits, size_t nlines, unsigned long long *__restrict__ count) {
    const size_t words = (nlines + 31) / 32;
    const uint32_t tail = (uint32_t)(nlines & 31u);
    unsigned long long n = 0;
    for (size_t w = (size_t)blockIdx.x * 256 + threadIdx.x; w < words; w += (size_t)gridDim.x * 256) {
        uint32_t v = bits[w];
        if (w + 1 == words && tail) v &= (1u << tail) - 1u;
        n += (uint32_t)__popc(v);
    }
    for (int d = 32; d > 0; d >>= 1) n += __shfl_down(n, d, 64);
    if ((threadIdx.x & 63) == 0 && n) atomicAdd(count, n);
}
int bitmap_count(const uint32_t *bits, size_t nlines, unsigned long long *count, void *stream) {
    hipError_t e = hipMemsetAsync(count, 0, sizeof *count, (hipStream_t)stream);
    if (e != hipSuccess || !nlines) return (int)e;
    size_t blocks = ((nlines + 31) / 32 + 255) / 256;
    if (blocks > 2048) blocks = 2048;
    hipLaunchKernelGGL(bitmap_count_kernel, dim3((unsigned)blocks), dim3(256), 0, (hipStream_t)stream, bits, nlines, count);
    return (int)hipGetLastError();
}
int mail_results(const uint64_t *total, const uint32_t *flags, const uint8_t *last_byte, uint64_t *mail, void *stream, const uint32_t *own) {
    hipLaunchKernelGGL(mail_results_kernel, dim3(1), dim3(64), 0, (hipStream_t)stream, total, flags, last_byte, mail, own);
    return (int)hipGetLastError();
}
int own_words_check(const uint64_t *stripe_base, size_t nstripes, const uint8_t *last_byte, uint32_t *own, void *stream) {
    const size_t nworkgroups = (nstripes + kThreads - 1) / kThreads;
    hipLaunchKernelGGL(own_words_kernel, dim3((unsigned)((nworkgroups + 255) / 256)), dim3(256), 0, (hipStream_t)stream, stripe_base, nstripes, nworkgroups,
                       last_byte, own);
    return (int)hipGetLastError();
}
int build_line_offsets(const uint8_t *bytes, size_t nbytes, uint32_t stripe, const uint64_t *stripe_base, size_t nstripes,
                       uint64_t *line_off, void *stream) {
    if (!nstripes) return 0;
    hipLaunchKernelGGL(line_offsets_kernel, dim3((unsigned)((nstripes + 255) / 256)), dim3(256), 0, (hipStream_t)stream, bytes, nbytes, stripe,
                       stripe_base, nstripes, line_off);
    return (int)hipGetLastError();
}
int empty_matches(const uint64_t *line_off, size_t nlines, uint32_t *count, const uint64_t *first, uint32_t *match_start, uint32_t *match_end,
                  void *stream, size_t cap) {
    if (!nlines) return 0;
    const dim3 grid((unsigned)((nlines + 255) / 256));
    if (first) hipLaunchKernelGGL(empty_matches_kernel<true>, grid, dim3(256), 0, (hipStream_t)stream, line_off, nlines, count, first, match_start, match_end, (uint64_t)cap);
    else hipLaunchKernelGGL(empty_matches_kernel<false>, grid, dim3(256), 0, (hipStream_t)stream, line_off, nlines, count, first, match_start, match_end, (uint64_t)cap);
    return (int)hipGetLastError();
}

}
}
```

### roaringregex_amd/csrc/kernels_nfa.inc

```
#include "item_lanes.hpp"

namespace rrx {
namespace dev {
namespace {

template <int W>
struct NfaCore {
    struct State { uint32_t s[W]; };
    const uint32_t *B;
    const uint32_t *X;
    NfaMasks m;
    bool any_exc, any_carry;

    static size_t lds_bytes(const NfaDevice &p) { return ((size_t)256 * W + (size_t)p.nbits * W) * 4; }
    __device__ void load(const NfaDevice &p, uint8_t *lds) {
        uint32_t *b = reinterpret_cast<uint32_t *>(lds);
        uint32_t *x = b + 256 * W;
        copy_table_to_lds(b, p.B, 256u * W * 4u);
        copy_table_to_lds(x, p.X, p.nbits * W * 4u);
        B = b; X = x; m = p.masks; any_exc = p.any_exc != 0; any_carry = p.any_carry != 0;
    }
    __device__ __forceinline__ bool accepting(const State &st) const {
        uint32_t a = 0;
#pragma unroll
        for (int i = 0; i < W; i++) a |= st.s[i] & m.fin[i];
        return a != 0;
    }
    __device__ __forceinline__ void advance(State &st, uint32_t c) const {
        uint32_t t[W];
        uint32_t exc = 0;
#pragma unroll
        for (int i = 0; i < W; i++) {
            uint32_t lo = i ? st.s[i - 1] : 0u;
            uint32_t sh = __builtin_amdgcn_alignbit(st.s[i], lo, 31);
            t[i] = (sh & m.chain[i]) | (st.s[i] & m.self[i]);
            exc |= st.s[i] & m.excm[i];
        }
        if (any_carry) {
            uint32_t cy = 0;
#pragma unroll
            for (int i = 0; i < W; i++) {
                const uint64_t sum = (uint64_t)(st.s[i] & m.cgrp[i]) + m.cgrp[i] + cy;
                t[i] |= (uint32_t)sum & m.ctgt[i];
                cy = (uint32_t)(sum >> 32);
            }
        }
        if (any_exc && exc) {
#pragma unroll
            for (int i = 0; i < W; i++) {
                uint32_t e = st.s[i] & m.excm[i];
                while (e) {
                    int b = __ffs(e) - 1;
                    e &= e - 1;
                    const uint32_t *row = X + (size_t)(32 * i + b) * W;
#pragma unroll
                    for (int j = 0; j < W; j++) t[j] |= row[j];
                }
            }
        }
        const uint32_t *bc = B + c * W;
#pragma unroll
        for (int i = 0; i < W; i++) st.s[i] = t[i] & bc[i];
    }
};

template <int W, bool SELF, bool RULES, bool CARRY = false>
struct LineNfaEngine : NfaCore<W> {
    static constexpr bool kStaged = !RULES;
    static constexpr bool kLdsAtZero = true;
    static constexpr bool kEightWaves = W <= 2 && !RULES;
    static constexpr int kRoundBytes = W <= 4 ? kRound : kRound / 2;
    using State = typename NfaCore<W>::State;
    __device__ void load(const NfaDevice &p, uint8_t *lds) {
        NfaCore<W>::load(p, lds);
        __syncthreads();
        uint32_t *b = reinterpret_cast<uint32_t *>(lds);
        if (threadIdx.x < W) b[(size_t)'\n' * W + threadIdx.x] = threadIdx.x == 0 ? 1u : 0u;
    }
    __device__ __forceinline__ State fresh() const {
        State st;
#pragma unroll
        for (int i = 0; i < W; i++) st.s[i] = i == 0 ? 1u : 0u;
        return st;
    }
    __device__ __forceinline__ State skipping() const {
        State st;
#pragma unroll
        for (int i = 0; i < W; i++) st.s[i] = 0;
        return st;
    }
    __device__ __forceinline__ void advance_line(State &st, uint32_t c) const { advance_row(st, this->B + c * W); }
    __device__ __forceinline__ void advance_row(State &st, const uint32_t *bc) const {
        uint32_t t[W];
        t[0] = (st.s[0] << 1) | 1u;
#pragma unroll
        for (int i = 1; i < W; i++) t[i] = __builtin_amdgcn_alignbit(st.s[i], st.s[i - 1], 31);
        if (SELF) {
#pragma unroll
            for (int i = 0; i < W; i++) t[i] |= st.s[i] & this->m.self[i];
        }
        if (RULES || CARRY) {
            if (CARRY || this->any_carry) {
                uint32_t cy = 0;
#pragma unroll
                for (int i = 0; i < W; i++) {
                    const uint64_t sum = (uint64_t)(st.s[i] & this->m.cgrp[i]) + this->m.cgrp[i] + cy;
                    t[i] |= (uint32_t)sum & this->m.ctgt[i];
                    cy = (uint32_t)(sum >> 32);
                }
            }
            if (RULES && this->any_exc) {
                uint32_t exc = 0;
#pragma unroll
                for (int i = 0; i < W; i++) exc |= st.s[i] & this->m.excm[i];
                if (exc) {
#pragma unroll
                    for (int i = 0; i < W; i++) {
                        uint32_t e = st.s[i] & this->m.excm[i];
                        while (e) {
                            const int b = __ffs(e) - 1;
                            e &= e - 1;
                            const uint32_t *row = this->X + (size_t)(32 * i + b) * W;
#pragma unroll
                            for (int j = 0; j < W; j++) t[j] |= row[j];
                        }
                    }
                }
            }
        }
#pragma unroll
        for (int i = 0; i < W; i++) st.s[i] = t[i] & bc[i];
    }
    typedef const __attribute__((address_space(3))) uint32_t *lds_u32_ptr;
    struct Row { uint32_t b[W]; };
    template <int K>
    __device__ __forceinline__ Row row_of(uint32_t w) const {
        uint32_t off;
        const uint32_t row_bytes = W * 4;
#define RRX_NFA_ROW(SEL) asm("v_mul_u32_u24_sdwa %0, %1, %2 dst_sel:DWORD dst_unused:UNUSED_PAD src0_sel:" SEL " src1_sel:DWORD" : "=v"(off) : "v"(w), "v"(row_bytes))
        if constexpr (K == 0) RRX_NFA_ROW("BYTE_0");
        if constexpr (K == 1) RRX_NFA_ROW("BYTE_1");
        if constexpr (K == 2) RRX_NFA_ROW("BYTE_2");
        if constexpr (K == 3) RRX_NFA_ROW("BYTE_3");
#undef RRX_NFA_ROW
        const lds_u32_ptr p = reinterpret_cast<lds_u32_ptr>(off);
        Row r;
#pragma unroll
        for (int i = 0; i < W; i++) r.b[i] = p[i];
        return r;
    }
    template <int K>
    __device__ __forceinline__ void verdict(const State &st, uint32_t w, uint32_t &bits) const {
        uint64_t nlmask;
        const uint32_t ten = '\n';
#define RRX_NFA_NL(SEL) asm("v_cmp_eq_u32_sdwa %0, %1, %2 src0_sel:" SEL " src1_sel:DWORD" : "=s"(nlmask) : "v"(w), "v"(ten))
        if constexpr (K == 0) RRX_NFA_NL("BYTE_0");
        if constexpr (K == 1) RRX_NFA_NL("BYTE_1");
        if constexpr (K == 2) RRX_NFA_NL("BYTE_2");
        if constexpr (K == 3) RRX_NFA_NL("BYTE_3");
#undef RRX_NFA_NL
        if (nlmask) {
            uint32_t a = 0, tmp;
#pragma unroll
            for (int i = 0; i < W; i++) a |= st.s[i] & this->m.fin[i];
            asm volatile("v_cmp_ne_u32_e32 vcc, 0, %2\n\t"
                         "v_addc_co_u32_e32 %1, vcc, %0, %0, vcc\n\t"
                         "v_cndmask_b32_e64 %0, %0, %1, %3"
                         : "+v"(bits), "=&v"(tmp) : "v"(a), "s"(nlmask) : "vcc");
        }
    }
    __device__ __forceinline__ void consume_word(State &st, uint32_t w, uint32_t &bits) const {
        if constexpr (W <= 4 && !RULES) {
            const Row r0 = row_of<0>(w), r1 = row_of<1>(w), r2 = row_of<2>(w), r3 = row_of<3>(w);
            verdict<0>(st, w, bits); advance_row(st, r0.b);
            verdict<1>(st, w, bits); advance_row(st, r1.b);
            verdict<2>(st, w, bits); advance_row(st, r2.b);
            verdict<3>(st, w, bits); advance_row(st, r3.b);
        } else {
            Row r = row_of<0>(w), n = row_of<1>(w);
            verdict<0>(st, w, bits); advance_row(st, r.b);
            r = row_of<2>(w);
            verdict<1>(st, w, bits); advance_row(st, n.b);
            n = row_of<3>(w);
            verdict<2>(st, w, bits); advance_row(st, r.b);
            verdict<3>(st, w, bits); advance_row(st, n.b);
        }
    }
    __device__ __forceinline__ void step(State &st, uint32_t c, uint32_t &nl, uint32_t &acc) const {
        const bool isnl = c == '\n';
        nl = isnl ? 1u : 0u;
        acc = (isnl && this->accepting(st)) ? 1u : 0u;
        advance_line(st, c);
    }
};

template <int W, bool RULES>
struct ContainsLineNfaEngine : LineNfaEngine<W, true, RULES, !RULES> {
    using Line = LineNfaEngine<W, true, RULES, !RULES>;
    static constexpr bool kStaged = Line::kStaged;
    static constexpr bool kLdsAtZero = true;
    static constexpr bool kEightWaves = W == 1 && !RULES;
    static constexpr int kRoundBytes = Line::kRoundBytes;
    struct State : NfaCore<W>::State { uint32_t found; };
    __device__ __forceinline__ State fresh() const {
        State st;
#pragma unroll
        for (int i = 0; i < W; i++) st.s[i] = i == 0 ? 1u : 0u;
        st.found = 0;
        return st;
    }
    __device__ __forceinline__ State skipping() const {
        State st;
#pragma unroll
        for (int i = 0; i < W; i++) st.s[i] = 0;
        st.found = 0;
        return st;
    }
    __device__ __forceinline__ void advance_found(State &st, const uint32_t *bc) const {
        this->advance_row(st, bc);
#pragma unroll
        for (int i = 0; i < W; i++) st.found = (st.s[i] & this->m.fin[i]) | st.found;
    }
    template <int K>
    __device__ __forceinline__ void verdict(State &st, uint32_t w, uint32_t &bits) const {
        uint64_t nlmask;
        const uint32_t ten = '\n';
#define RRX_NFA_NL(SEL) asm("v_cmp_eq_u32_sdwa %0, %1, %2 src0_sel:" SEL " src1_sel:DWORD" : "=s"(nlmask) : "v"(w), "v"(ten))
        if constexpr (K == 0) RRX_NFA_NL("BYTE_0");
        if constexpr (K == 1) RRX_NFA_NL("BYTE_1");
        if constexpr (K == 2) RRX_NFA_NL("BYTE_2");
        if constexpr (K == 3) RRX_NFA_NL("BYTE_3");
#undef RRX_NFA_NL
        if (nlmask) {
            uint32_t tmp;
            asm volatile("v_cmp_ne_u32_e32 vcc, 0, %1\n\t"
                         "v_addc_co_u32_e32 %2, vcc, %0, %0, vcc\n\t"
                         "v_cndmask_b32_e64 %0, %0, %2, %3\n\t"
                         "v_cndmask_b32_e64 %1, %1, 0, %3"
                         : "+v"(bits), "+v"(st.found), "=&v"(tmp) : "s"(nlmask) : "vcc");
        }
    }
    __device__ __forceinline__ void consume_word(State &st, uint32_t w, uint32_t &bits) const {
        using Row = typename Line::Row;
        if constexpr (W <= 4 && !RULES) {
            const Row r0 = this->template row_of<0>(w), r1 = this->template row_of<1>(w), r2 = this->template row_of<2>(w), r3 = this->template row_of<3>(w);
            verdict<0>(st, w, bits); advance_found(st, r0.b);
            verdict<1>(st, w, bits); advance_found(st, r1.b);
            verdict<2>(st, w, bits); advance_found(st, r2.b);
            verdict<3>(st, w, bits); advance_found(st, r3.b);
        } else {
            Row r = this->template row_of<0>(w), n = this->template row_of<1>(w);
            verdict<0>(st, w, bits); advance_found(st, r.b);
            r = this->template row_of<2>(w);
            verdict<1>(st, w, bits); advance_found(st, n.b);
            n = this->template row_of<3>(w);
            verdict<2>(st, w, bits); advance_found(st, r.b);
            verdict<3>(st, w, bits); advance_found(st, n.b);
        }
    }
    __device__ __forceinline__ void step(State &st, uint32_t c, uint32_t &nl, uint32_t &acc) const {
        const bool isnl = c == '\n';
        nl = isnl ? 1u : 0u;
        acc = (isnl && st.found) ? 1u : 0u;
        if (isnl) st.found = 0;
        advance_found(st, this->B + c * W);
    }
};

template <int W>
struct PlainNfaEngine : NfaCore<W> {
    using State = typename NfaCore<W>::State;
    __device__ __forceinline__ void reset(State &st) const {
#pragma unroll
        for (int i = 0; i < W; i++) st.s[i] = this->m.init[i];
    }
    __device__ __forceinline__ void kill(State &st) const {
#pragma unroll
        for (int i = 0; i < W; i++) st.s[i] = 0;
    }
    __device__ __forceinline__ void step(State &st, uint32_t c) const { this->advance(st, c); }
};

template <int W>
__global__ __launch_bounds__(kThreads) void contains_extents_nfa_kernel(NfaDevice prog, const uint8_t *__restrict__ bytes,
                                                                         const uint64_t *__restrict__ off, size_t nitems, uint32_t trim,
                                                                         uint32_t *__restrict__ bits) {
    extern __shared__ __attribute__((aligned(16))) uint8_t smem[];
    NfaCore<W> eng;
    eng.load(prog, smem);
    __syncthreads();
    for_each_wave_pass(nitems, [&](size_t first, uint32_t lane) {
        const size_t i = first + lane;
        bool hit = false;
        if (i < nitems) {
            const auto [b, e] = item_span(off, i, trim);
            typename NfaCore<W>::State st;
#pragma unroll
            for (int k = 0; k < W; k++) st.s[k] = eng.m.init[k];
            hit = eng.accepting(st);
            size_t p = b;
            auto one = [&](uint32_t c) {
                eng.advance(st, c);
#pragma unroll
                for (int k = 0; k < W; k++) st.s[k] |= eng.m.init[k];
                hit = eng.accepting(st);
            };
            for (; p < e && (p & 15) && !hit; p++) one(bytes[p]);
            for (; p + 16 <= e && !hit; p += 16) {
                const uint4 v = *reinterpret_cast<const uint4 *>(bytes + p);
                const uint32_t w[4] = {v.x, v.y, v.z, v.w};
#pragma unroll
                for (int k = 0; k < 16; k++)
                    if (!hit) one((w[k >> 2] >> (8 * (k & 3))) & 0xffu);
            }
            for (; p < e && !hit; p++) one(bytes[p]);
        }
        const uint64_t verdicts = __builtin_amdgcn_ballot_w64(hit);
        if (lane == 0) {
            bits[first >> 5] = (uint32_t)verdicts;
            if (first + 32 < nitems) bits[(first >> 5) + 1] = (uint32_t)(verdicts >> 32);
        }
    });
}

template <int W>
__global__ __launch_bounds__(256) void long_rows_nfa_kernel(NfaDevice prog, const uint8_t *__restrict__ bytes, size_t nbytes, uint32_t chunk,
                                                             uint32_t nchunks, uint32_t *__restrict__ rows) {
    extern __shared__ __attribute__((aligned(16))) uint8_t smem[];
    PlainNfaEngine<W> eng;
    eng.load(prog, smem);
    __syncthreads();
    const uint32_t N = prog.nbits;
    const size_t item = (size_t)blockIdx.x * 256 + threadIdx.x;
    if (item >= (size_t)nchunks * N) return;
    const size_t k = item / N;
    const uint32_t p = (uint32_t)(item % N);
    const size_t a = k * (size_t)chunk, b = a + chunk < nbytes ? a + chunk : nbytes;
    typename PlainNfaEngine<W>::State st;
#pragma unroll
    for (int i = 0; i < W; i++) st.s[i] = (uint32_t)i == (p >> 5) ? 1u << (p & 31) : 0u;
    auto alive = [&]() { uint32_t o = 0; for (int i = 0; i < W; i++) o |= st.s[i]; return o != 0; };
    size_t pos = a;
    if ((reinterpret_cast<uintptr_t>(bytes + pos) & 15) == 0) {
        for (; pos + 16 <= b && alive(); pos += 16) {
            const uint4 v = *reinterpret_cast<const uint4 *>(bytes + pos);
            const uint32_t w[4] = {v.x, v.y, v.z, v.w};
#pragma unroll
            for (int i = 0; i < 16; i++) {
                const uint32_t c = (w[i >> 2] >> (8 * (i & 3))) & 0xffu;
                if (c == 0 || c >= 0x80) eng.kill(st); else eng.step(st, c);
            }
        }
    }
    for (; pos < b && alive(); pos++) { const uint32_t c = bytes[pos]; if (c == 0 || c >= 0x80) eng.kill(st); else eng.step(st, c); }
#pragma unroll
    for (int i = 0; i < W; i++) rows[item * W + i] = st.s[i];
}
template <int W>
__global__ __launch_bounds__(256) void long_compose_nfa_kernel(const uint32_t *__restrict__ in, uint32_t nin, uint32_t N, uint32_t *__restrict__ out) {
    const size_t item = (size_t)blockIdx.x * 256 + threadIdx.x;
    const uint32_t nout = (nin + 1) / 2;
    if (item >= (size_t)nout * N) return;
    const size_t k = item / N;
    const uint32_t *a = in + ((size_t)2 * k * N + item % N) * W;
    uint32_t acc[W];
    if (2 * k + 1 >= nin) {
#pragma unroll
        for (int i = 0; i < W; i++) acc[i] = a[i];
    } else {
        const uint32_t *bm = in + (size_t)(2 * k + 1) * N * W;
#pragma unroll
        for (int i = 0; i < W; i++) acc[i] = 0;
#pragma unroll
        for (int i = 0; i < W; i++) {
            uint32_t e = a[i];
            while (e) {
                const uint32_t q = 32u * i + (uint32_t)__ffs(e) - 1u;
                e &= e - 1;
                const uint32_t *row = bm + (size_t)q * W;
#pragma unroll
                for (int j = 0; j < W; j++) acc[j] |= row[j];
            }
        }
    }
#pragma unroll
    for (int i = 0; i < W; i++) out[item * W + i] = acc[i];
}
template <int W>
__global__ void long_finish_nfa_kernel(NfaDevice prog, const uint32_t *__restrict__ rel, uint8_t *__restrict__ accept) {
    if (threadIdx.x || blockIdx.x) return;
    uint32_t a = 0;
    for (int i = 0; i < W; i++) {
        uint32_t e = prog.masks.init[i];
        while (e) {
            const uint32_t q = 32u * i + (uint32_t)__ffs(e) - 1u;
            e &= e - 1;
            for (int j = 0; j < W; j++) a |= rel[(size_t)q * W + j] & prog.masks.fin[j];
        }
    }
    accept[0] = a ? 1 : 0;
}

template <int W>
__global__ __launch_bounds__(256) void recheck_escaped_kernel(NfaDevice prog, const uint8_t *__restrict__ bytes, size_t nbytes, uint32_t stripe,
                                                               const uint64_t *__restrict__ stripe_base, size_t nstripes,
                                                               const uint32_t *__restrict__ escaped_bits, uint32_t *__restrict__ accept_bits,
                                                               const unsigned long long *__restrict__ escaped_total, size_t cap) {
    extern __shared__ __attribute__((aligned(16))) uint8_t smem[];
    if (*escaped_total <= cap) return;
    PlainNfaEngine<W> eng;
    eng.load(prog, smem);
    __syncthreads();
    const size_t g = (size_t)blockIdx.x * 256 + threadIdx.x;
    if (g >= nstripes) return;
    const uint64_t b0 = stripe_base[g], b1 = stripe_base[g + 1];
    const bool next_fresh = g + 1 < nstripes ? (b1 & kFreshStripe) != 0 : bytes[nbytes - 1] == '\n';
    const uint64_t lo = line_of(b0) + ((b0 & kFreshStripe) ? 0u : 1u);
    const uint64_t past = line_of(b1) + (next_fresh ? 0u : 1u);
    if (past <= lo) return;
    auto escaped = [&](uint64_t line) -> bool { return (escaped_bits[line >> 5] >> (line & 31u)) & 1u; };
    uint64_t last = past;
    for (uint64_t w = lo >> 5; w <= (past - 1) >> 5; w++) {
        uint32_t m = escaped_bits[w];
        if (w == lo >> 5) m &= ~0u << (lo & 31u);
        if (w == (past - 1) >> 5 && ((past - 1) & 31u) != 31u) m &= (2u << ((past - 1) & 31u)) - 1u;
        if (m) last = w * 32 + (31u - (uint32_t)__clz((int)m));
    }
    if (last == past) return;
    size_t pos = g * (size_t)stripe;
    uint4 buf = make_uint4(0, 0, 0, 0);
    size_t buf_at = ~(size_t)0;
    auto byte_at = [&](size_t q) -> uint32_t {
        const size_t a = q & ~(size_t)15;
        if (a != buf_at) {
            buf_at = a;
            if (a + 16 <= nbytes) buf = *reinterpret_cast<const uint4 *>(bytes + a);
            else {
                uint32_t w4[4] = {0, 0, 0, 0};
                for (size_t k = a; k < nbytes; k++) w4[(k - a) >> 2] |= (uint32_t)bytes[k] << (8 * ((k - a) & 3));
                buf = make_uint4(w4[0], w4[1], w4[2], w4[3]);
            }
        }
        const uint32_t k = (uint32_t)(q & 15);
        const uint32_t word = k < 4 ? buf.x : k < 8 ? buf.y : k < 12 ? buf.z : buf.w;
        return (word >> (8 * (k & 3))) & 0xffu;
    };
    auto skip_line = [&]() { while (pos < nbytes && byte_at(pos++) != '\n') {} };
    uint64_t line = lo;
    if (!(b0 & kFreshStripe)) skip_line();
    for (; line <= last && pos <= nbytes; line++) {
        if (!escaped(line)) { skip_line(); continue; }
        typename PlainNfaEngine<W>::State st;
        eng.reset(st);
        bool dead = false;
        while (pos < nbytes) {
            const uint32_t c = byte_at(pos++);
            if (c == '\n') break;
            if (dead) continue;
            if (c == 0 || c >= 0x80) { eng.kill(st); dead = true; } else eng.step(st, c);
        }
        if (!dead && eng.accepting(st)) atomicOr(&accept_bits[line >> 5], 1u << (line & 31u));
    }
}

template <int W>
__global__ __launch_bounds__(256) void recheck_lines_kernel(NfaDevice prog, const uint8_t *__restrict__ bytes, size_t nbytes, uint32_t stripe,
                                                             const uint64_t *__restrict__ stripe_base, size_t nstripes, const uint64_t *__restrict__ list,
                                                             const unsigned long long *__restrict__ escaped_total, size_t cap, uint32_t *__restrict__ accept_bits) {
    extern __shared__ __attribute__((aligned(16))) uint8_t smem[];
    const unsigned long long total = *escaped_total;
    if (!total || total > cap) return;
    PlainNfaEngine<W> eng;
    eng.load(prog, smem);
    __syncthreads();
    uint4 buf = make_uint4(0, 0, 0, 0);
    size_t buf_at = ~(size_t)0;
    auto chunk_at = [&](size_t a) -> uint4 {
        if (a + 16 <= nbytes) return *reinterpret_cast<const uint4 *>(bytes + a);
        uint32_t w4[4] = {0, 0, 0, 0};
        for (size_t k = a; k < nbytes; k++) w4[(k - a) >> 2] |= (uint32_t)bytes[k] << (8 * ((k - a) & 3));
        return make_uint4(w4[0], w4[1], w4[2], w4[3]);
    };
    auto byte_at = [&](size_t q) -> uint32_t {
        const size_t a = q & ~(size_t)15;
        if (a != buf_at) { buf_at = a; buf = chunk_at(a); }
        const uint32_t k = (uint32_t)(q & 15);
        const uint32_t word = k < 4 ? buf.x : k < 8 ? buf.y : k < 12 ? buf.z : buf.w;
        return (word >> (8 * (k & 3))) & 0xffu;
    };
    auto newlines_in = [](uint32_t w) -> uint32_t {
        const uint32_t t = w ^ 0x0a0a0a0au;
        return ~(((t & 0x7f7f7f7fu) + 0x7f7f7f7fu) | t) & 0x80808080u;
    };
    for (size_t j = (size_t)blockIdx.x * 256 + threadIdx.x; j < total; j += (size_t)gridDim.x * 256) {
        const uint64_t line = list[j];
        size_t pos = 0;
        if (line) {
            size_t lo = 0, hi = nstripes;
            while (hi - lo > 1) {
                const size_t mid = lo + (hi - lo) / 2;
                if (line_of(stripe_base[mid]) < line) lo = mid; else hi = mid;
            }
            uint32_t need = (uint32_t)(line - line_of(stripe_base[lo]));
            pos = lo * (size_t)stripe;
            while (pos + 64 <= nbytes) {
                const uint4 *q4 = reinterpret_cast<const uint4 *>(bytes + pos);
                const uint4 v0 = q4[0], v1 = q4[1], v2 = q4[2], v3 = q4[3];
                const uint32_t c = (uint32_t)(__popc(newlines_in(v0.x)) + __popc(newlines_in(v0.y)) + __popc(newlines_in(v0.z)) + __popc(newlines_in(v0.w)) +
                                              __popc(newlines_in(v1.x)) + __popc(newlines_in(v1.y)) + __popc(newlines_in(v1.z)) + __popc(newlines_in(v1.w)) +
                                              __popc(newlines_in(v2.x)) + __popc(newlines_in(v2.y)) + __popc(newlines_in(v2.z)) + __popc(newlines_in(v2.w)) +
                                              __popc(newlines_in(v3.x)) + __popc(newlines_in(v3.y)) + __popc(newlines_in(v3.z)) + __popc(newlines_in(v3.w)));
                if (c >= need) break;
                need -= c;
                pos += 64;
            }
            while (pos < nbytes) {
                const uint4 v = chunk_at(pos);
                const uint32_t f[4] = {newlines_in(v.x), newlines_in(v.y), newlines_in(v.z), newlines_in(v.w)};
                const uint32_t c = (uint32_t)(__popc(f[0]) + __popc(f[1]) + __popc(f[2]) + __popc(f[3]));
                if (c < need) { need -= c; pos += 16; continue; }
                for (int q = 0; q < 4; q++) {
                    uint32_t m = f[q];
                    while (m) {
                        const uint32_t bit = (uint32_t)__ffs((int)m) - 1u;
                        m &= m - 1;
                        if (--need == 0) { pos += 4u * q + (bit >> 3) + 1u; q = 4; break; }
                    }
                }
                break;
            }
        }
        typename PlainNfaEngine<W>::State st;
        eng.reset(st);
        bool dead = false;
        while (pos < nbytes) {
            const uint32_t c = byte_at(pos++);
            if (c == '\n') break;
            if (dead) break;
            if (c == 0 || c >= 0x80) { eng.kill(st); dead = true; } else eng.step(st, c);
        }
        if (!dead && eng.accepting(st)) atomicOr(&accept_bits[line >> 5], 1u << (line & 31u));
    }
}

}

#if RRX_NFA_PART == 0
#define RRX_NFA_DISPATCH(CALL) switch (p.W) { case 1: return CALL(1); case 2: return CALL(2); default: return (int)hipErrorInvalidValue; }
#define RRX_NFA_NAME(base) base##_part0
#elif RRX_NFA_PART == 1
#define RRX_NFA_DISPATCH(CALL) switch (p.W) { case 3: return CALL(3); case 4: return CALL(4); default: return (int)hipErrorInvalidValue; }
#define RRX_NFA_NAME(base) base##_part1
#elif RRX_NFA_PART == 2
#define RRX_NFA_DISPATCH(CALL) switch (p.W) { case 5: case 6: return CALL(6); case 7: case 8: return CALL(8); default: return (int)hipErrorInvalidValue; }
#define RRX_NFA_NAME(base) base##_part2
#else
#define RRX_NFA_DISPATCH(CALL) switch (p.W) { case 9: case 10: case 11: case 12: return CALL(12); case 13: case 14: case 15: case 16: return CALL(16); default: return (int)hipErrorInvalidValue; }
#define RRX_NFA_NAME(base) base##_part3
#endif

int RRX_NFA_NAME(match_stripes_nfa)(const NfaDevice &p, const uint8_t *bytes, size_t nbytes, uint32_t stripe, const uint64_t *stripe_base,
                                    size_t nstripes, uint32_t *accept, void *stream) {
#define GO(WW, S, R, C) launch_stripes<LineNfaEngine<WW, S, R, C>, NfaDevice>(p, LineNfaEngine<WW, S, R, C>::lds_bytes(p), bytes, nbytes, stripe, stripe_base, nstripes, accept, stream)
#define CALL(WW) (p.any_exc ? GO(WW, true, true, false) : p.any_carry ? GO(WW, true, false, true) : p.any_self ? GO(WW, true, false, false) : GO(WW, false, false, false))
    RRX_NFA_DISPATCH(CALL)
#undef CALL
#undef GO
}
int RRX_NFA_NAME(match_onepass_nfa)(const NfaDevice &p, const uint8_t *bytes, size_t nbytes, uint32_t stripe, size_t nstripes, uint32_t *counts,
                                    uint32_t *slabs, void *stream) {
#define GO(WW, S, R, C) launch_onepass<LineNfaEngine<WW, S, R, C>, NfaDevice>(p, LineNfaEngine<WW, S, R, C>::lds_bytes(p), bytes, nbytes, stripe, nstripes, counts, slabs, stream)
#define CALL(WW) (p.any_exc ? GO(WW, true, true, false) : (p.any_self || p.any_carry) ? GO(WW, true, false, true) : GO(WW, false, false, false))
    RRX_NFA_DISPATCH(CALL)
#undef CALL
#undef GO
}
int RRX_NFA_NAME(match_long_nfa)(const NfaDevice &p, const uint8_t *bytes, size_t nbytes, uint32_t chunk, uint32_t nchunks, void *scratch,
                                 uint8_t *accept, void *stream) {
#define CALL(WW) [&]() -> int {                                                                                                  \
        const size_t lds = PlainNfaEngine<WW>::lds_bytes(p);                                                                       \
        static LdsAttr attr;                                                                                                        \
        hipError_t e = ensure_dynamic_lds(attr, reinterpret_cast<const void *>(long_rows_nfa_kernel<WW>), lds);                   \
        if (e != hipSuccess) return (int)e;                                                                                         \
        const size_t items = (size_t)nchunks * p.nbits;                                                                             \
        hipLaunchKernelGGL(long_rows_nfa_kernel<WW>, dim3((unsigned)((items + 255) / 256)), dim3(256), lds, (hipStream_t)stream, p, bytes, nbytes, chunk, \
                           nchunks, static_cast<uint32_t *>(scratch));                                                             \
        uint32_t *cur = static_cast<uint32_t *>(scratch), *other = cur + items * WW;       \
        for (uint32_t n = nchunks; n > 1; n = (n + 1) / 2) {                                                                       \
            const size_t out_items = (size_t)((n + 1) / 2) * p.nbits;                                                              \
            hipLaunchKernelGGL(long_compose_nfa_kernel<WW>, dim3((unsigned)((out_items + 255) / 256)), dim3(256), 0, (hipStream_t)stream, cur, n, p.nbits, other); \
            uint32_t *tmp = cur; cur = other; other = tmp;                                                                          \
        }                                                                                                                           \
        hipLaunchKernelGGL(long_finish_nfa_kernel<WW>, dim3(1), dim3(64), 0, (hipStream_t)stream, p, cur, accept);               \
        return (int)hipGetLastError();                                                                                              \
    }()
    RRX_NFA_DISPATCH(CALL)
#undef CALL
}
int RRX_NFA_NAME(recheck_escaped_nfa)(const NfaDevice &p, const uint8_t *bytes, size_t nbytes, uint32_t stripe, const uint64_t *stripe_base, size_t nstripes,
                                      const uint32_t *escaped_bits, size_t nlines, const uint64_t *list, const unsigned long long *escaped_total, size_t cap,
                                      uint32_t *accept_bits, void *stream) {
#define CALL(WW) [&]() -> int {                                                                                                  \
        const size_t lds = PlainNfaEngine<WW>::lds_bytes(p);                                                                       \
        if (!nstripes || !nlines) return 0;                                                                                         \
        static LdsAttr attr, attr2;                                                                                                 \
        hipError_t e = ensure_dynamic_lds(attr, reinterpret_cast<const void *>(recheck_lines_kernel<WW>), lds);                   \
        if (e == hipSuccess) e = ensure_dynamic_lds(attr2, reinterpret_cast<const void *>(recheck_escaped_kernel<WW>), lds);      \
        if (e != hipSuccess) return (int)e;                                                                                         \
                                                   \
        hipLaunchKernelGGL(recheck_lines_kernel<WW>, dim3(1024), dim3(256), lds, (hipStream_t)stream, p, bytes, nbytes, stripe, stripe_base, nstripes, list,   \
                           escaped_total, cap, accept_bits);                                                                       \
                                 \
        hipLaunchKernelGGL(recheck_escaped_kernel<WW>, dim3((unsigned)((nstripes + 255) / 256)), dim3(256), lds, (hipStream_t)stream, p, bytes, nbytes, stripe, \
                           stripe_base, nstripes, escaped_bits, accept_bits, escaped_total, cap);                                  \
        return (int)hipGetLastError();                                                                                              \
    }()
    RRX_NFA_DISPATCH(CALL)
#undef CALL
}
int RRX_NFA_NAME(match_extents_nfa)(const NfaDevice &p, const uint8_t *bytes, const uint64_t *off, size_t nitems, uint32_t trim, uint8_t *accept,
                                    void *stream) {
#define CALL(WW) launch_extents<PlainNfaEngine<WW>, NfaDevice>(p, PlainNfaEngine<WW>::lds_bytes(p), bytes, off, nitems, trim, accept, stream)
    RRX_NFA_DISPATCH(CALL)
#undef CALL
}
int RRX_NFA_NAME(contains_stripes_nfa)(const NfaDevice &p, const uint8_t *bytes, size_t nbytes, uint32_t stripe, const uint64_t *stripe_base,
                                       size_t nstripes, uint32_t *bits, void *stream) {
#define GO(WW, R) launch_stripes<ContainsLineNfaEngine<WW, R>, NfaDevice>(p, ContainsLineNfaEngine<WW, R>::lds_bytes(p), bytes, nbytes, stripe, stripe_base, nstripes, bits, stream)
#define CALL(WW) (p.any_exc ? GO(WW, true) : GO(WW, false))
    RRX_NFA_DISPATCH(CALL)
#undef CALL
#undef GO
}
int RRX_NFA_NAME(contains_extents_nfa)(const NfaDevice &p, const uint8_t *bytes, const uint64_t *off, size_t nitems, uint32_t trim, uint32_t *bits,
                                       void *stream) {
    if (!nitems) return 0;
#define CALL(WW) launch_item_lanes<contains_extents_nfa_kernel<WW>>(NfaCore<WW>::lds_bytes(p), nitems, kItemLanesMaxBlocks, stream, p, bytes, off, nitems, trim, bits)
    RRX_NFA_DISPATCH(CALL)
#undef CALL
}
}
}
```

### roaringregex_amd/csrc/kernels_table.hip

```cpp
#include "item_lanes.hpp"

namespace rrx {
namespace dev {
namespace {

struct NoPhaseHook { __device__ __forceinline__ void operator()(int) const {} __device__ __forceinline__ void round(int) const {} };
enum { kPhaseEntry = 0, kPhaseTablesLoaded, kPhaseFirstRound, kPhaseMainDone, kPhaseFollowDone, kPhaseWindowOut, kPhases };
__device__ __forceinline__ void feed_load(uint4 (&buf)[kRound / 16], const uint4 *p) {
#pragma unroll
    for (int i = 0; i < kRound / 16; i++) buf[i] = load_text(p + i);
    asm volatile("" : : "v"(p));
}
template <bool ONEPASS, class PhaseHook, int FLUSH_SLOTS, int KB = 1, bool CLEAN = ONEPASS, class Engine = Dfa2>
__device__ __forceinline__ void dfa2_stripe(const Engine &eng, const size_t g, const uint64_t window_word, uint32_t *const stage, const uint32_t stage_words,
                                            const uint8_t *__restrict__ bytes, const size_t nbytes, const uint32_t stripe,
                                            const uint64_t *__restrict__ stripe_base, uint32_t *__restrict__ accept_bits,
                                            uint32_t *__restrict__ counts, uint32_t *__restrict__ slabs, const uint32_t slab_row, PhaseHook &phase,
                                            const uint32_t flush_mask) {
    static_assert(FLUSH_SLOTS >= 0 && (FLUSH_SLOTS & (FLUSH_SLOTS - 1)) == 0, "0 or a power of two");
    const size_t start = g * (size_t)stripe;
    if (start < nbytes) {
    const size_t stripe_end = start + stripe;
    const size_t my_end = stripe_end < nbytes ? stripe_end : nbytes;
    bool fresh = true;
    typename std::conditional<ONEPASS, LocalResults, ResultsT<true>>::type res;
    if constexpr (ONEPASS) {
        res.begin(slabs + g, slab_row);
    } else {
        const uint64_t my_base = stripe_base[g];
        fresh = (my_base & kFreshStripe) != 0;
        res.begin_staged(line_of(my_base) * KB, window_word, !fresh, accept_bits, stage);
        res.stage_words = stage_words;
        res.drop_mask = (1u << KB) - 1u;
    }
    typename Engine::State st = fresh ? eng.fresh() : eng.skipping();
    auto clean = [](uint32_t w) -> uint32_t {
        if (CLEAN && __builtin_amdgcn_ballot_w64((w & 0x80808080u) != 0)) {
            const uint32_t hi = (w & 0x80808080u) >> 7;
            w &= ~(hi * 0xffu);
        }
        return w;
    };

    size_t pos = start;
    const uint4 *src = reinterpret_cast<const uint4 *>(bytes + start);
    constexpr int kSlots = kRound / 16;
    const int rounds = (int)((my_end - start) / kRound);
    uint4 buf[kSlots];
    if (rounds > 0) feed_load(buf, src);
    uint32_t last_word = 0;
    bool ahead = false;
    for (int r = 0; r < rounds; r++) {
        if (r == 1) phase(kPhaseFirstRound);
        phase.round(r);
#pragma unroll
        for (int i = 0; i < kSlots; i++) {
            if (CLEAN && __builtin_expect(__builtin_amdgcn_ballot_w64(((buf[i].x | buf[i].y | buf[i].z | buf[i].w) & 0x80808080u) != 0) != 0, 0)) {
                eng.consume_dword(st, clean(buf[i].x), res.bits);
                eng.consume_dword(st, clean(buf[i].y), res.bits);
                eng.consume_dword(st, clean(buf[i].z), res.bits);
                eng.consume_dword(st, clean(buf[i].w), res.bits);
            } else {
                eng.consume_dword(st, buf[i].x, res.bits);
                eng.consume_dword(st, buf[i].y, res.bits);
                if (KB == 2 && (res.bits >> 15)) res.flush();
                eng.consume_dword(st, buf[i].z, res.bits);
                eng.consume_dword(st, buf[i].w, res.bits);
            }
            bool together;
            if constexpr (FLUSH_SLOTS == 0) together = (((uint32_t)r * kSlots + (uint32_t)i) & flush_mask) == flush_mask;
            else if constexpr (FLUSH_SLOTS >= kSlots) together = i == kSlots - 1 && (r & (FLUSH_SLOTS / kSlots - 1)) == FLUSH_SLOTS / kSlots - 1;
            else together = (i & (FLUSH_SLOTS - 1)) == FLUSH_SLOTS - 1;
            if (together) res.flush();
            else if (res.bits >> 15) res.flush();
        }
        if (r + 1 < rounds) {
            feed_load(buf, src + (r + 1) * kSlots);
        } else {
            last_word = buf[kSlots - 1].w;
            if (start + (size_t)(rounds + 1) * kRound <= nbytes) {
                feed_load(buf, src + (r + 1) * kSlots);
                ahead = true;
            }
        }
    }
    pos += (size_t)rounds * kRound;
    phase(kPhaseMainDone);
    auto byte_at = [&](size_t q) -> uint32_t { const uint32_t b = bytes[q]; return (CLEAN && b >= 0x80u) ? 0u : b; };

    bool closed_by_end_of_data = false;
    for (; pos + 2 <= my_end; pos += 2) {
        uint32_t lines, verdicts;
        eng.step2(st, byte_at(pos), byte_at(pos + 1), lines, verdicts);
        res.bits = (res.bits << lines) | verdicts;
        if (res.bits >> (31 - 2 * KB)) res.flush();
    }
    if (pos < my_end) {
        const uint32_t b = byte_at(pos);
        uint32_t lines, verdicts;
        eng.step2(st, b, '\n', lines, verdicts);
        if (b == '\n') res.push(KB, verdicts >> KB);
        else { res.push(KB, verdicts); closed_by_end_of_data = true; }
        pos++;
    }
    res.flush();
    const uint32_t newlines = res.seen - (closed_by_end_of_data ? 1u : 0u);

    if (ONEPASS && res.seen == 0) fresh = g == 0 || bytes[start - 1] == '\n';
    const bool started = fresh || res.seen > 0;
    bool followed = false;
    const bool whole_rounds = rounds > 0 && start + (size_t)rounds * kRound == my_end;
    const uint32_t last_byte = whole_rounds ? last_word >> 24 : (uint32_t)bytes[my_end - 1];
    if (!closed_by_end_of_data && started && last_byte != '\n') {
        uint32_t lines = 0, verdicts = 0;
        if (ahead && pos == start + (size_t)(rounds + 1) * kRound - kRound) {
    #pragma unroll
            for (int i = 0; i < kSlots; i++) {
                if (!lines) {
                    const uint32_t w[4] = {clean(buf[i].x), clean(buf[i].y), clean(buf[i].z), clean(buf[i].w)};
#pragma unroll
                    for (int k = 0; k < 8; k++)
                        if (!lines) eng.step2(st, (w[k >> 1] >> (16 * (k & 1))) & 0xffu, (w[k >> 1] >> (16 * (k & 1) + 8)) & 0xffu, lines, verdicts);
                    pos += 16;
                }
            }
        }
        while (pos + 16 <= nbytes && !lines) {
            const uint4 v = *reinterpret_cast<const uint4 *>(bytes + pos);
            const uint32_t w[4] = {clean(v.x), clean(v.y), clean(v.z), clean(v.w)};
#pragma unroll
            for (int k = 0; k < 8; k++)
                if (!lines) eng.step2(st, (w[k >> 1] >> (16 * (k & 1))) & 0xffu, (w[k >> 1] >> (16 * (k & 1) + 8)) & 0xffu, lines, verdicts);
            pos += 16;
        }
        for (; pos + 2 <= nbytes && !lines; pos += 2) eng.step2(st, byte_at(pos), byte_at(pos + 1), lines, verdicts);
        if (!lines) eng.step2(st, pos < nbytes ? byte_at(pos) : '\n', '\n', lines, verdicts);
        res.push(KB, lines == 2 * KB ? verdicts >> KB : verdicts);
        followed = true;
    }
    res.finish();
    phase(kPhaseFollowDone);
    if (ONEPASS)
        counts[g] = newlines | ((followed || closed_by_end_of_data) ? kExtraResult : 0u) | (last_byte == '\n' ? kEndsOnNewline : 0u);
    }
}

__device__ __forceinline__ void settle_shared_word(unsigned long long *slot, uint32_t *word, uint32_t mine) {
    const unsigned long long old = atomicExch(slot, (1ull << 63) | mine);
    if (old) {
        *word = (uint32_t)old | mine;
        *slot = 0;
    }
}
template <bool ONEPASS, int FLUSH_SLOTS, class PhaseHook = NoPhaseHook, int KB = 1, bool CLEAN = ONEPASS, bool OWN_WORDS = false, bool PAIRS8 = false>
__device__ __forceinline__ void dfa2_body(const Dfa2Device &prog, const uint8_t *__restrict__ bytes, size_t nbytes, uint32_t stripe,
                                          const uint64_t *__restrict__ stripe_base, uint32_t *__restrict__ accept_bits,
                                          uint32_t *__restrict__ counts, uint32_t *__restrict__ slabs, PhaseHook phase = PhaseHook(),
                                          uint32_t flush_mask = 31u, unsigned long long *__restrict__ slots = nullptr, uint64_t nwords = 0) {
    static_assert(!OWN_WORDS || (!ONEPASS && KB == 1), "the exchange slots serve the indexed kernels with one bit per line");
    phase(kPhaseEntry);
    __shared__ __attribute__((aligned(16))) struct {
        uint8_t t2_and_stage[kDfa2RegionBytes];
        uint8_t p[Dfa2T<PAIRS8>::kPBytes];
    } lds;
    Dfa2T<PAIRS8> eng;
    eng.load(prog, lds.p, lds.t2_and_stage);
    const uint32_t stage_off = (uint32_t)((Dfa2::lds_bytes(prog) + 15) & ~(size_t)15);
    uint32_t *const stage = reinterpret_cast<uint32_t *>(lds.t2_and_stage + stage_off);
    const uint32_t stage_words = (kDfa2RegionBytes - stage_off) / 4;
    if (!ONEPASS)
        for (uint32_t i = threadIdx.x; i < stage_words; i += kThreads) stage[i] = 0;
    __syncthreads();
    phase(kPhaseTablesLoaded);

    const size_t g0 = (size_t)blockIdx.x * kThreads;
    uint64_t window_word = 0;
    if (!ONEPASS) window_word = (line_of(stripe_base[g0]) * KB) >> 5;
    dfa2_stripe<ONEPASS, PhaseHook, FLUSH_SLOTS, KB, CLEAN, Dfa2T<PAIRS8>>(eng, g0 + threadIdx.x, window_word, stage, stage_words, bytes, nbytes, stripe, stripe_base, accept_bits,
                                                            counts, slabs, gridDim.x * kThreads, phase, flush_mask);
    if constexpr (OWN_WORDS) {
        __syncthreads();
        const bool last = blockIdx.x + 1 == gridDim.x;
        const uint64_t next_word = last ? nwords : line_of(stripe_base[g0 + kThreads]) >> 5;
        uint64_t span = next_word - window_word;
        if (span > stage_words) span = stage_words;
        for (uint32_t i = threadIdx.x + 1; i < (uint32_t)span; i += kThreads) accept_bits[window_word + i] = stage[i];
        if (threadIdx.x == 0) {
            if (blockIdx.x == 0) accept_bits[window_word] = stage[0];
            else settle_shared_word(&slots[blockIdx.x], &accept_bits[window_word], stage[0]);
        }
        if (threadIdx.x == 64 && !last && span < stage_words) settle_shared_word(&slots[blockIdx.x + 1], &accept_bits[next_word], stage[(uint32_t)span]);
    } else if (!ONEPASS) {
        __syncthreads();
        for (uint32_t i = threadIdx.x; i < stage_words; i += kThreads) {
            const uint32_t v = stage[i];
            if (v) atomicOr(&accept_bits[window_word + i], v);
        }
    }
    phase(kPhaseWindowOut);
}
template <int FLUSH_SLOTS, bool OWN_WORDS, bool PAIRS8>
__global__ __launch_bounds__(kThreads) void match_stripes2_kernel(Dfa2Device prog, const uint8_t *__restrict__ bytes, size_t nbytes,
                                                                   uint32_t stripe, const uint64_t *__restrict__ stripe_base,
                                                                   uint32_t *__restrict__ accept_bits, uint32_t flush_mask,
                                                                   unsigned long long *__restrict__ slots, uint64_t nwords) {
    dfa2_body<false, FLUSH_SLOTS, NoPhaseHook, 1, false, OWN_WORDS, PAIRS8>(prog, bytes, nbytes, stripe, stripe_base, accept_bits, nullptr, nullptr, NoPhaseHook(), flush_mask,
                                                                    slots, nwords);
}
template <int FLUSH_SLOTS, bool OWN_WORDS, bool PAIRS8>
__global__ __launch_bounds__(kThreads) void match_stripes2_clean_kernel(
    Dfa2Device prog, const uint8_t *__restrict__ bytes, size_t nbytes, uint32_t stripe, const uint64_t *__restrict__ stripe_base,
    uint32_t *__restrict__ accept_bits, uint32_t flush_mask, unsigned long long *__restrict__ slots, uint64_t nwords) {
    dfa2_body<false, FLUSH_SLOTS, NoPhaseHook, 1, true, OWN_WORDS, PAIRS8>(prog, bytes, nbytes, stripe, stripe_base, accept_bits, nullptr, nullptr, NoPhaseHook(), flush_mask,
                                                                   slots, nwords);
}
__global__ __launch_bounds__(kThreads) void match_stripes2_two_bit_kernel(Dfa2Device prog, const uint8_t *__restrict__ bytes, size_t nbytes,
                                                                           uint32_t stripe, const uint64_t *__restrict__ stripe_base,
                                                                           uint32_t *__restrict__ wide_bits) {
    dfa2_body<false, 32, NoPhaseHook, 2>(prog, bytes, nbytes, stripe, stripe_base, wide_bits, nullptr, nullptr);
}
__global__ __launch_bounds__(kThreads) void match_stripes2_onepass_kernel(Dfa2Device prog, const uint8_t *__restrict__ bytes, size_t nbytes,
                                                                           uint32_t stripe, uint32_t *__restrict__ counts,
                                                                           uint32_t *__restrict__ slabs) {
    dfa2_body<true, 32>(prog, bytes, nbytes, stripe, nullptr, nullptr, counts, slabs);
}

constexpr uint32_t kCompactWindowWords = 8192;
__global__ __launch_bounds__(256) void compact_streams_kernel(const uint32_t *__restrict__ counts, const uint64_t *__restrict__ stripe_base,
                                                               size_t nstripes, uint32_t stripe, const uint32_t *__restrict__ slabs,
                                                               uint32_t *__restrict__ accept_bits, size_t cap_words) {
    __shared__ uint32_t window[kCompactWindowWords];
    const size_t g0 = (size_t)blockIdx.x * 256;
    const size_t g1 = g0 + 256 < nstripes ? g0 + 256 : nstripes;
    const uint64_t window_word = line_of(stripe_base[g0]) >> 5;
    const uint64_t span = (line_of(stripe_base[g1]) >> 5) - window_word + 2;
    const uint32_t used = span < kCompactWindowWords ? (uint32_t)span : kCompactWindowWords;
    for (uint32_t i = threadIdx.x; i < used; i += 256) window[i] = 0;
    __syncthreads();
    const size_t g = g0 + threadIdx.x;
    if (g < nstripes) {
        const uint32_t c = counts[g];
        const uint32_t n = (c & kCountMask) + ((c & kExtraResult) ? 1u : 0u);
        const uint64_t b = stripe_base[g];
        const uint64_t base = line_of(b);
        const bool fresh = (b & kFreshStripe) != 0;
        const size_t row = (nstripes + kThreads - 1) / kThreads * kThreads;
        const uint32_t *src = slabs + g;
        auto put = [&](uint64_t word, uint32_t v) {
            if (!v) return;
            if (word >= cap_words) return;
            const uint64_t rel = word - window_word;
            if (rel < used) atomicOr(&window[(uint32_t)rel], v);
            else atomicOr(&accept_bits[word], v);
        };
        for (uint32_t k = 0; k * 32 < n; k++) {
            uint32_t v = src[(size_t)k * row];
            if (n - k * 32 < 32) v &= (1u << (n - k * 32)) - 1u;
            if (k == 0 && !fresh) v &= ~1u;
            const uint64_t bit = base + (uint64_t)k * 32;
            const uint32_t sh = (uint32_t)bit & 31u;
            put(bit >> 5, v << sh);
            if (sh) put((bit >> 5) + 1, v >> (32u - sh));
        }
    }
    __syncthreads();
    for (uint32_t i = threadIdx.x; i < used; i += 256) {
        const uint32_t v = window[i];
        if (v && window_word + i < cap_words) atomicOr(&accept_bits[window_word + i], v);
    }
}

}

int match_stripes_dfa(const LineDfaDevice &p, bool clamp_high, const uint8_t *bytes, size_t nbytes, uint32_t stripe,
                      const uint64_t *stripe_base, size_t nstripes, uint32_t *accept, void *stream) {
#define GO(WIDE, CLAMP) launch_stripes<LineDfaEngine<WIDE, CLAMP>, LineDfaDevice>(p, LineDfaEngine<WIDE, CLAMP>::lds_bytes(p), bytes, nbytes, stripe, stripe_base, nstripes, accept, stream)
    if (p.in_global) return launch_stripes<LineDfaGlobalEngine, LineDfaDevice>(p, 256, bytes, nbytes, stripe, stripe_base, nstripes, accept, stream);
    if (p.wide) return clamp_high ? GO(true, true) : GO(true, false);
    return GO(false, false);
#undef GO
}
uint32_t flush_mask_for(size_t nbytes, size_t nlines) {
    const size_t avg = nlines ? nbytes / nlines : nbytes;
    uint32_t slots = 1;
    while (slots < 32 && (size_t)slots * 2 * 16 <= avg * 16) slots *= 2;
    return slots - 1;
}
template <class... Params, class... Rest>
static int launch_dfa2(void (*kernel)(Params...), const Dfa2Device &p, const uint8_t *bytes, size_t nbytes, uint32_t stripe, size_t nstripes,
                       size_t stripes_per_wg, void *stream, Rest... rest) {
    if (!nstripes) return 0;
    if (Dfa2::lds_bytes(p) > kDfa2MaxTable) return (int)hipErrorInvalidValue;
    const size_t blocks = (nstripes + stripes_per_wg - 1) / stripes_per_wg;
    hipLaunchKernelGGL(kernel, dim3((unsigned)blocks), dim3(kThreads), 0, (hipStream_t)stream, p, bytes, nbytes, stripe, rest...);
    return (int)hipGetLastError();
}
uint32_t dfa2_window_words(const Dfa2Device &p) {
    const size_t stage_off = (Dfa2::lds_bytes(p) + 15) & ~(size_t)15;
    return stage_off < kDfa2RegionBytes ? (uint32_t)((kDfa2RegionBytes - stage_off) / 4) : 0u;
}
bool dfa2_flush_at_compile_time(uint32_t flush_mask) { return flush_mask == 31u; }
template <bool PAIRS8>
static int launch_match_stripes2(const Dfa2Device &p, bool clean, const uint8_t *bytes, size_t nbytes, uint32_t stripe, const uint64_t *stripe_base,
                                 size_t nstripes, uint32_t *accept, void *stream, uint32_t flush_mask, unsigned long long *slots, size_t nwords) {
    const bool fixed = dfa2_flush_at_compile_time(flush_mask);
#define GO(K) launch_dfa2(K, p, bytes, nbytes, stripe, nstripes, kThreads, stream, stripe_base, accept, flush_mask, slots, (uint64_t)nwords)
    if (clean) {
        if (slots) return fixed ? GO((match_stripes2_clean_kernel<32, true, PAIRS8>)) : GO((match_stripes2_clean_kernel<0, true, PAIRS8>));
        return fixed ? GO((match_stripes2_clean_kernel<32, false, PAIRS8>)) : GO((match_stripes2_clean_kernel<0, false, PAIRS8>));
    }
    if (slots) return fixed ? GO((match_stripes2_kernel<32, true, PAIRS8>)) : GO((match_stripes2_kernel<0, true, PAIRS8>));
    return fixed ? GO((match_stripes2_kernel<32, false, PAIRS8>)) : GO((match_stripes2_kernel<0, false, PAIRS8>));
#undef GO
}
int match_stripes_dfa2(const Dfa2Device &p, bool clean, const uint8_t *bytes, size_t nbytes, uint32_t stripe, const uint64_t *stripe_base,
                       size_t nstripes, uint32_t *accept, void *stream, uint32_t flush_mask, unsigned long long *slots, size_t nwords) {
    return p.P8 ? launch_match_stripes2<true>(p, clean, bytes, nbytes, stripe, stripe_base, nstripes, accept, stream, flush_mask, slots, nwords)
                : launch_match_stripes2<false>(p, clean, bytes, nbytes, stripe, stripe_base, nstripes, accept, stream, flush_mask, slots, nwords);
}
__global__ __launch_bounds__(256) void split_two_bit_kernel(const uint32_t *__restrict__ wide, size_t words, uint32_t *__restrict__ accept_bits,
                                                             uint32_t *__restrict__ escaped_bits, unsigned long long *__restrict__ escaped_total,
                                                             uint64_t *__restrict__ list, size_t cap) {
    constexpr uint32_t kLocal = 4096, kFlushAt = kLocal - 256 * 8;
    __shared__ uint64_t local[kLocal];
    __shared__ uint32_t nlocal;
    __shared__ unsigned long long flush_base;
    if (threadIdx.x == 0) nlocal = 0;
    __syncthreads();
    auto even_bits = [](uint32_t x) -> uint32_t {
        x &= 0x55555555u;
        x = (x | x >> 1) & 0x33333333u;
        x = (x | x >> 2) & 0x0f0f0f0fu;
        x = (x | x >> 4) & 0x00ff00ffu;
        return (x | x >> 8) & 0xffffu;
    };
    auto flush = [&]() {
        __syncthreads();
        const uint32_t n = nlocal;
        if (n) {
            if (threadIdx.x == 0) flush_base = atomicAdd(escaped_total, (unsigned long long)n);
            __syncthreads();
            const unsigned long long base = flush_base;
            for (uint32_t i = threadIdx.x; i < n; i += 256) if (base + i < cap) list[base + i] = local[i];
            __syncthreads();
            if (threadIdx.x == 0) nlocal = 0;
        }
        __syncthreads();
    };
    const size_t turns = (words + (size_t)gridDim.x * 256 - 1) / ((size_t)gridDim.x * 256);
    for (size_t it = 0; it < turns; it++) {
        const size_t w = (it * gridDim.x + blockIdx.x) * 256 + threadIdx.x;
        uint32_t esc = 0;
        if (w < words) {
            const uint2 v = reinterpret_cast<const uint2 *>(wide)[w];
            accept_bits[w] = even_bits(v.x) | even_bits(v.y) << 16;
            esc = even_bits(v.x >> 1) | even_bits(v.y >> 1) << 16;
            escaped_bits[w] = esc;
        }
        while (__syncthreads_or(esc != 0)) {
            uint32_t take = 0;
            for (uint32_t k = 0, m = esc; k < 8 && m; k++) { take |= m & (0u - m); m &= m - 1; }
            const uint32_t c = (uint32_t)__popc(take);
            if (c) {
                uint32_t at = atomicAdd(&nlocal, c);
                for (uint32_t m = take; m; m &= m - 1) local[at++] = (uint64_t)w * 32 + (uint32_t)(__ffs((int)m) - 1);
            }
            esc &= ~take;
            __syncthreads();
            if (nlocal > kFlushAt) flush();
        }
    }
    flush();
}
int match_stripes_dfa2_two_bit(const Dfa2Device &p, const uint8_t *bytes, size_t nbytes, uint32_t stripe, const uint64_t *stripe_base,
                               size_t nstripes, uint32_t *wide_bits, void *stream) {
    return launch_dfa2(match_stripes2_two_bit_kernel, p, bytes, nbytes, stripe, nstripes, kThreads, stream, stripe_base, wide_bits);
}
int split_two_bit(const uint32_t *wide, size_t nlines, uint32_t *accept_bits, uint32_t *escaped_bits, unsigned long long *escaped_total, uint64_t *list,
                  size_t cap, void *stream) {
    const size_t words = (nlines + 31) / 32;
    if (!words) return 0;
    size_t blocks = (words + 255) / 256;
    if (blocks > 2048) blocks = 2048;
    hipLaunchKernelGGL(split_two_bit_kernel, dim3((unsigned)blocks), dim3(256), 0, (hipStream_t)stream, wide, words, accept_bits, escaped_bits, escaped_total,
                       list, cap);
    return (int)hipGetLastError();
}
int match_onepass_dfa(const LineDfaDevice &p, const uint8_t *bytes, size_t nbytes, uint32_t stripe, size_t nstripes, uint32_t *counts,
                      uint32_t *slabs, void *stream) {
    if (p.in_global) return launch_onepass<LineDfaGlobalEngine, LineDfaDevice>(p, 256, bytes, nbytes, stripe, nstripes, counts, slabs, stream);
    if (p.wide) return launch_onepass<LineDfaEngine<true, true>, LineDfaDevice>(p, LineDfaEngine<true, true>::lds_bytes(p), bytes, nbytes, stripe, nstripes, counts, slabs, stream);
    return launch_onepass<LineDfaEngine<false, false>, LineDfaDevice>(p, LineDfaEngine<false, false>::lds_bytes(p), bytes, nbytes, stripe, nstripes, counts, slabs, stream);
}
size_t onepass_slab_words(size_t nstripes, uint32_t stripe) {
    return ((nstripes + kThreads - 1) / kThreads) * slab_words_per_lane(stripe) * kThreads;
}
int match_onepass_dfa2(const Dfa2Device &p, const uint8_t *bytes, size_t nbytes, uint32_t stripe, size_t nstripes, uint32_t *counts,
                       uint32_t *slabs, void *stream) {
    return launch_dfa2(match_stripes2_onepass_kernel, p, bytes, nbytes, stripe, nstripes, kThreads, stream, counts, slabs);
}
int compact_streams(const uint32_t *counts, const uint64_t *stripe_base, size_t nstripes, uint32_t stripe, const uint32_t *slabs,
                    uint32_t *accept_bits, size_t cap_words, void *stream) {
    if (!nstripes) return 0;
    hipLaunchKernelGGL(compact_streams_kernel, dim3((unsigned)((nstripes + 255) / 256)), dim3(256), 0, (hipStream_t)stream, counts, stripe_base, nstripes,
                       stripe, slabs, accept_bits, cap_words);
    return (int)hipGetLastError();
}
int match_extents_dfa(const DfaDevice &p, const uint8_t *bytes, const uint64_t *off, size_t nitems, uint32_t trim, uint8_t *accept,
                      void *stream, const uint32_t *only_if) {
    if (PlainDfaEngine::lds_bytes(p) > kPlainDfaLdsBudget)
        return launch_extents<PlainDfaGlobalEngine, DfaDevice>(p, PlainDfaGlobalEngine::lds_bytes(p), bytes, off, nitems, trim, accept, stream, only_if);
    return launch_extents<PlainDfaEngine, DfaDevice>(p, PlainDfaEngine::lds_bytes(p), bytes, off, nitems, trim, accept, stream, only_if);
}

}
}
```

Measured before the change: 5654.

## Fold stripe-count scan into match and compact kernels, drop separate scan and mail launches

The one-pass match kernel now reduces per-block newline totals into a small totals array. The compaction kernel computes each block's base with its own decoupled prefix over earlier block totals and a block-level exclusive scan, instead of relying on a separate scan_counts kernel. The mailbox write is folded into the last compaction block. This removes two kernel launches and the 64-bit stripe_base array, at the cost of each compact block re-summing all preceding block totals and using a larger 1024-thread workgroup with dynamic LDS. It also templates the dfa2 onepass kernel on PAIRS8.

```diff
diff --git a/roaringregex_amd/csrc/corpus.cpp b/roaringregex_amd/csrc/corpus.cpp
--- a/roaringregex_amd/csrc/corpus.cpp
+++ b/roaringregex_amd/csrc/corpus.cpp
@@ -283,27 +283,25 @@
     const uint8_t *bytes = static_cast<const uint8_t *>(d_bytes);
     const uint32_t stripe = dev::pick_stripe(nbytes);
     const size_t nstripes = (nbytes + stripe - 1) / stripe;
-    const size_t counts_bytes = ((nstripes + 2) * sizeof(uint32_t) + 15) & ~(size_t)15;
-    const size_t base_bytes = (nstripes + 1 + dev::scan_scratch_words(nstripes)) * sizeof(uint64_t);
+    const size_t counts_bytes = (nstripes * sizeof(uint32_t) + 15) & ~(size_t)15;
+    const size_t totals_bytes = (dev::onepass_total_words(nstripes) * sizeof(uint32_t) + 15) & ~(size_t)15;
     const size_t slab_bytes = dev::onepass_slab_words(nstripes, stripe) * sizeof(uint32_t);
     std::lock_guard<std::mutex> lock(re->onepass_mu);
     void *buf = nullptr;
-    rc = re->onepass_for(device, counts_bytes + base_bytes + slab_bytes, &buf, st);
+    rc = re->onepass_for(device, counts_bytes + totals_bytes + slab_bytes, &buf, st);
     if (rc) return rc;
     uint32_t *d_counts = static_cast<uint32_t *>(buf);
-    uint64_t *d_base = reinterpret_cast<uint64_t *>(static_cast<uint8_t *>(buf) + counts_bytes);
-    uint32_t *d_slabs = reinterpret_cast<uint32_t *>(static_cast<uint8_t *>(buf) + counts_bytes + base_bytes);
+    uint32_t *d_totals = reinterpret_cast<uint32_t *>(static_cast<uint8_t *>(buf) + counts_bytes);
+    uint32_t *d_slabs = reinterpret_cast<uint32_t *>(static_cast<uint8_t *>(buf) + counts_bytes + totals_bytes);
     MailboxGuard mail;
     rc = mailbox_acquire(device, &mail.m);
     if (rc) return rc;
     if (cap_words) HIP_TRY(hipMemsetAsync(d_accept_bits, 0, cap_words * sizeof(uint32_t), st));
-    int e = re->engine == RRX_ENGINE_NFA ? dev::match_onepass_nfa(t->nfa, bytes, nbytes, stripe, nstripes, d_counts, d_slabs, stream)
-            : re->match.has_dfa2         ? dev::match_onepass_dfa2(re->dfa2_device(t), bytes, nbytes, stripe, nstripes, d_counts, d_slabs, stream)
-                                         : dev::match_onepass_dfa(t->line, bytes, nbytes, stripe, nstripes, d_counts, d_slabs, stream);
-    if (!e) e = dev::scan_counts(d_counts, d_base, d_base + nstripes + 1, nstripes, stream);
-    if (!e) e = dev::compact_streams(d_counts, d_base, nstripes, stripe, d_slabs, d_accept_bits, cap_words, stream);
+    int e = re->engine == RRX_ENGINE_NFA ? dev::match_onepass_nfa(t->nfa, bytes, nbytes, stripe, nstripes, d_counts, d_slabs, d_totals, stream)
+            : re->match.has_dfa2         ? dev::match_onepass_dfa2(re->dfa2_device(t), bytes, nbytes, stripe, nstripes, d_counts, d_slabs, d_totals, stream)
+                                         : dev::match_onepass_dfa(t->line, bytes, nbytes, stripe, nstripes, d_counts, d_slabs, d_totals, stream);
     mail.stream = st; mail.queued = true;
-    if (!e) e = dev::mail_results(d_base + nstripes, nullptr, bytes + nbytes - 1, mail.m.dev, stream);
+    if (!e) e = dev::compact_streams(d_counts, d_totals, nstripes, stripe, d_slabs, d_accept_bits, cap_words, bytes + nbytes - 1, mail.m.dev, stream);
     if (e) return hip_fail((hipError_t)e, "one-pass launch");
     const hipError_t he = hipStreamSynchronize(st);
     if (he != hipSuccess) return hip_fail(he, "one-pass readback");
diff --git a/roaringregex_amd/csrc/device.hpp b/roaringregex_amd/csrc/device.hpp
--- a/roaringregex_amd/csrc/device.hpp
+++ b/roaringregex_amd/csrc/device.hpp
@@ -124,12 +124,13 @@
                   size_t cap, void *stream);
 
 size_t onepass_slab_words(size_t nstripes, uint32_t stripe);
+size_t onepass_total_words(size_t nstripes);
 int match_onepass_dfa2(const Dfa2Device &p, const uint8_t *bytes, size_t nbytes, uint32_t stripe, size_t nstripes, uint32_t *counts,
-                       uint32_t *slabs, void *stream);
+                       uint32_t *slabs, uint32_t *totals, void *stream);
 int match_onepass_dfa(const LineDfaDevice &p, const uint8_t *bytes, size_t nbytes, uint32_t stripe, size_t nstripes, uint32_t *counts,
-                      uint32_t *slabs, void *stream);
-int compact_streams(const uint32_t *counts, const uint64_t *stripe_base, size_t nstripes, uint32_t stripe, const uint32_t *slabs,
-                    uint32_t *accept_bits, size_t cap_words, void *stream);
+                      uint32_t *slabs, uint32_t *totals, void *stream);
+int compact_streams(const uint32_t *counts, const uint32_t *totals, size_t nstripes, uint32_t stripe, const uint32_t *slabs,
+                    uint32_t *accept_bits, size_t cap_words, const uint8_t *last_byte, uint64_t *mail, void *stream);
 int match_extents_dfa(const DfaDevice &p, const uint8_t *bytes, const uint64_t *off, size_t nitems, uint32_t trim,
                       uint8_t *accept, void *stream, const uint32_t *only_if = nullptr);
 
@@ -292,7 +293,7 @@
 int match_stripes_nfa(const NfaDevice &p, const uint8_t *bytes, size_t nbytes, uint32_t stripe, const uint64_t *stripe_base,
                       size_t nstripes, uint32_t *accept_bits, void *stream);
 int match_onepass_nfa(const NfaDevice &p, const uint8_t *bytes, size_t nbytes, uint32_t stripe, size_t nstripes, uint32_t *counts,
-                      uint32_t *slabs, void *stream);
+                      uint32_t *slabs, uint32_t *totals, void *stream);
 int recheck_escaped_nfa(const NfaDevice &p, const uint8_t *bytes, size_t nbytes, uint32_t stripe, const uint64_t *stripe_base, size_t nstripes,
                         const uint32_t *escaped_bits, size_t nlines, const uint64_t *list, const unsigned long long *escaped_total, size_t cap,
                         uint32_t *accept_bits, void *stream);
diff --git a/roaringregex_amd/csrc/kernels_common.hpp b/roaringregex_amd/csrc/kernels_common.hpp
--- a/roaringregex_amd/csrc/kernels_common.hpp
+++ b/roaringregex_amd/csrc/kernels_common.hpp
@@ -146,11 +146,50 @@
 constexpr uint32_t kExtraResult = 0x40000000u;
 __host__ __device__ inline size_t slab_words_per_lane(uint32_t stripe) { return stripe / 32 + 1; }
 
+template <int NW>
+__device__ __forceinline__ uint64_t block_exclusive_scan(uint64_t v, uint64_t *wave_tot, uint64_t &total) {
+    const int lane = threadIdx.x & 63, wave = threadIdx.x >> 6;
+    uint64_t inc = v;
+#pragma unroll
+    for (int d = 1; d < 64; d <<= 1) {
+        const uint64_t o = __shfl_up(inc, d, 64);
+        if (lane >= d) inc += o;
+    }
+    if (lane == 63) wave_tot[wave] = inc;
+    __syncthreads();
+    uint64_t off = 0, tot = 0;
+#pragma unroll
+    for (int w = 0; w < NW; w++) {
+        const uint64_t t = wave_tot[w];
+        if (w < wave) off += t;
+        tot += t;
+    }
+    total = tot;
+    return off + inc - v;
+}
+
+__device__ __forceinline__ uint32_t workgroup_wave() { return (uint32_t)__builtin_amdgcn_readfirstlane((int)(threadIdx.x >> 6)); }
+__device__ __forceinline__ void store_workgroup_total(uint32_t mine, uint32_t wave, uint32_t *lds, uint32_t *__restrict__ totals) {
+#pragma unroll
+    for (int d = 32; d; d >>= 1) mine += __shfl_xor(mine, d, 64);
+    const bool first_lane = __lane_id() == 0;
+    __syncthreads();
+    if (first_lane) lds[wave] = mine;
+    __syncthreads();
+    if (first_lane && wave == 0) {
+        uint32_t sum = 0;
+#pragma unroll
+        for (int w = 0; w < kThreads / 64; w++) sum += lds[w];
+        totals[blockIdx.x] = sum;
+    }
+}
+
 template <class Engine, class Program, bool ONEPASS = false>
 __device__ __forceinline__ void match_stripes_body(const Program &prog, const uint8_t *__restrict__ bytes, size_t nbytes,
                                                    uint32_t stripe, const uint64_t *__restrict__ stripe_base,
                                                    uint32_t *__restrict__ accept_bits, uint32_t stage_off, uint32_t stage_words,
-                                                   uint32_t *__restrict__ counts = nullptr, uint32_t *__restrict__ slabs = nullptr) {
+                                                   uint32_t *__restrict__ counts = nullptr, uint32_t *__restrict__ slabs = nullptr,
+                                                   uint32_t *__restrict__ totals = nullptr) {
     extern __shared__ __attribute__((aligned(16))) uint8_t smem[];
     constexpr bool kWindow = Engine::kStaged && !ONEPASS;
     uint32_t *stage = reinterpret_cast<uint32_t *>(smem + stage_off);
@@ -165,6 +204,8 @@
     if (!ONEPASS) window_word = line_of(stripe_base[g0]) >> 5;
     const size_t g = g0 + threadIdx.x;
     const size_t start = g * (size_t)stripe;
+    const uint32_t wave = workgroup_wave();
+    uint32_t my_newlines = 0;
     if (start < nbytes) {
     const size_t stripe_end = start + stripe;
     const size_t my_end = stripe_end < nbytes ? stripe_end : nbytes;
@@ -227,7 +268,9 @@
     }
     res.finish();
     if (ONEPASS) counts[g] = newlines | (followed ? kExtraResult : 0u) | (bytes[my_end - 1] == '\n' ? kEndsOnNewline : 0u);
-    }
+    my_newlines = newlines;
+    }
+    if constexpr (ONEPASS) store_workgroup_total(my_newlines, wave, reinterpret_cast<uint32_t *>(smem), totals);
     if (kWindow) {
         __syncthreads();
         for (uint32_t i = threadIdx.x; i < stage_words; i += kThreads) {
@@ -253,8 +296,9 @@
 }
 template <class Engine, class Program>
 __global__ __launch_bounds__(kThreads) void match_stripes_onepass_kernel(Program prog, const uint8_t *__restrict__ bytes, size_t nbytes, uint32_t stripe,
-                                                                          uint32_t *__restrict__ counts, uint32_t *__restrict__ slabs) {
-    match_stripes_body<Engine, Program, true>(prog, bytes, nbytes, stripe, nullptr, nullptr, 0, 0, counts, slabs);
+                                                                          uint32_t *__restrict__ counts, uint32_t *__restrict__ slabs,
+                                                                          uint32_t *__restrict__ totals) {
+    match_stripes_body<Engine, Program, true>(prog, bytes, nbytes, stripe, nullptr, nullptr, 0, 0, counts, slabs, totals);
 }
 constexpr int kMaxDevices = 64;
 struct LdsAttr { std::atomic<int> bytes[kMaxDevices]; std::atomic<int> at_zero_ok{0}; };
@@ -299,14 +343,15 @@
 
 template <class Engine, class Program>
 int launch_onepass(const Program &p, size_t table_bytes, const uint8_t *bytes, size_t nbytes, uint32_t stripe, size_t nstripes, uint32_t *counts,
-                   uint32_t *slabs, void *stream) {
+                   uint32_t *slabs, uint32_t *totals, void *stream) {
     if (!nstripes) return 0;
     auto k = match_stripes_onepass_kernel<Engine, Program>;
     static LdsAttr attr;
+    if (table_bytes < kThreads / 64 * sizeof(uint32_t)) table_bytes = kThreads / 64 * sizeof(uint32_t);
     hipError_t e = ensure_dynamic_lds(attr, reinterpret_cast<const void *>(k), table_bytes, lds_at_zero<Engine>::value);
     if (e != hipSuccess) return (int)e;
     size_t blocks = (nstripes + kThreads - 1) / kThreads;
-    hipLaunchKernelGGL(k, dim3((unsigned)blocks), dim3(kThreads), table_bytes, (hipStream_t)stream, p, bytes, nbytes, stripe, counts, slabs);
+    hipLaunchKernelGGL(k, dim3((unsigned)blocks), dim3(kThreads), table_bytes, (hipStream_t)stream, p, bytes, nbytes, stripe, counts, slabs, totals);
     return (int)hipGetLastError();
 }
 
diff --git a/roaringregex_amd/csrc/kernels_coop.hip b/roaringregex_amd/csrc/kernels_coop.hip
--- a/roaringregex_amd/csrc/kernels_coop.hip
+++ b/roaringregex_amd/csrc/kernels_coop.hip
@@ -296,8 +296,8 @@
               (const NfaDevice &p, const uint8_t *bytes, size_t nbytes, uint32_t stripe, const uint64_t *stripe_base, size_t nstripes, uint32_t *accept, void *stream),
               (p, bytes, nbytes, stripe, stripe_base, nstripes, accept, stream))
 RRX_NFA_PARTS(match_onepass_nfa,
-              (const NfaDevice &p, const uint8_t *bytes, size_t nbytes, uint32_t stripe, size_t nstripes, uint32_t *counts, uint32_t *slabs, void *stream),
-              (p, bytes, nbytes, stripe, nstripes, counts, slabs, stream))
+              (const NfaDevice &p, const uint8_t *bytes, size_t nbytes, uint32_t stripe, size_t nstripes, uint32_t *counts, uint32_t *slabs, uint32_t *totals, void *stream),
+              (p, bytes, nbytes, stripe, nstripes, counts, slabs, totals, stream))
 RRX_NFA_PARTS(match_extents_nfa,
               (const NfaDevice &p, const uint8_t *bytes, const uint64_t *off, size_t nitems, uint32_t trim, uint8_t *accept, void *stream),
               (p, bytes, off, nitems, trim, accept, stream))
diff --git a/roaringregex_amd/csrc/kernels_index.hip b/roaringregex_amd/csrc/kernels_index.hip
--- a/roaringregex_amd/csrc/kernels_index.hip
+++ b/roaringregex_amd/csrc/kernels_index.hip
@@ -140,27 +140,6 @@
     __syncthreads();
     if (threadIdx.x == 0) sums[blockIdx.x] = part[0] + part[1] + part[2] + part[3];
 }
-template <int NW>
-__device__ __forceinline__ uint64_t block_exclusive_scan(uint64_t v, uint64_t *wave_tot, uint64_t &total) {
-    const int lane = threadIdx.x & 63, wave = threadIdx.x >> 6;
-    uint64_t inc = v;
-#pragma unroll
-    for (int d = 1; d < 64; d <<= 1) {
-        const uint64_t o = __shfl_up(inc, d, 64);
-        if (lane >= d) inc += o;
-    }
-    if (lane == 63) wave_tot[wave] = inc;
-    __syncthreads();
-    uint64_t off = 0, tot = 0;
-#pragma unroll
-    for (int w = 0; w < NW; w++) {
-        const uint64_t t = wave_tot[w];
-        if (w < wave) off += t;
-        tot += t;
-    }
-    total = tot;
-    return off + inc - v;
-}
 __global__ __launch_bounds__(1024) void scan_sums_kernel(uint64_t *__restrict__ sums, size_t nchunks, uint64_t *__restrict__ total) {
     __shared__ uint64_t wave_tot[16];
     const size_t per = (nchunks + 1023) / 1024;
diff --git a/roaringregex_amd/csrc/kernels_nfa.inc b/roaringregex_amd/csrc/kernels_nfa.inc
--- a/roaringregex_amd/csrc/kernels_nfa.inc
+++ b/roaringregex_amd/csrc/kernels_nfa.inc
@@ -568,8 +568,8 @@
 #undef GO
 }
 int RRX_NFA_NAME(match_onepass_nfa)(const NfaDevice &p, const uint8_t *bytes, size_t nbytes, uint32_t stripe, size_t nstripes, uint32_t *counts,
-                                    uint32_t *slabs, void *stream) {
-#define GO(WW, S, R, C) launch_onepass<LineNfaEngine<WW, S, R, C>, NfaDevice>(p, LineNfaEngine<WW, S, R, C>::lds_bytes(p), bytes, nbytes, stripe, nstripes, counts, slabs, stream)
+                                    uint32_t *slabs, uint32_t *totals, void *stream) {
+#define GO(WW, S, R, C) launch_onepass<LineNfaEngine<WW, S, R, C>, NfaDevice>(p, LineNfaEngine<WW, S, R, C>::lds_bytes(p), bytes, nbytes, stripe, nstripes, counts, slabs, totals, stream)
 #define CALL(WW) (p.any_exc ? GO(WW, true, true, false) : (p.any_self || p.any_carry) ? GO(WW, true, false, true) : GO(WW, false, false, false))
     RRX_NFA_DISPATCH(CALL)
 #undef CALL
diff --git a/roaringregex_amd/csrc/kernels_table.hip b/roaringregex_amd/csrc/kernels_table.hip
--- a/roaringregex_amd/csrc/kernels_table.hip
+++ b/roaringregex_amd/csrc/kernels_table.hip
@@ -12,13 +12,14 @@
     asm volatile("" : : "v"(p));
 }
 template <bool ONEPASS, class PhaseHook, int FLUSH_SLOTS, int KB = 1, bool CLEAN = ONEPASS, class Engine = Dfa2>
-__device__ __forceinline__ void dfa2_stripe(const Engine &eng, const size_t g, const uint64_t window_word, uint32_t *const stage, const uint32_t stage_words,
+__device__ __forceinline__ uint32_t dfa2_stripe(const Engine &eng, const size_t g, const uint64_t window_word, uint32_t *const stage, const uint32_t stage_words,
                                             const uint8_t *__restrict__ bytes, const size_t nbytes, const uint32_t stripe,
                                             const uint64_t *__restrict__ stripe_base, uint32_t *__restrict__ accept_bits,
                                             uint32_t *__restrict__ counts, uint32_t *__restrict__ slabs, const uint32_t slab_row, PhaseHook &phase,
                                             const uint32_t flush_mask) {
     static_assert(FLUSH_SLOTS >= 0 && (FLUSH_SLOTS & (FLUSH_SLOTS - 1)) == 0, "0 or a power of two");
     const size_t start = g * (size_t)stripe;
+    uint32_t my_newlines = 0;
     if (start < nbytes) {
     const size_t stripe_end = start + stripe;
     const size_t my_end = stripe_end < nbytes ? stripe_end : nbytes;
@@ -142,7 +143,9 @@
     phase(kPhaseFollowDone);
     if (ONEPASS)
         counts[g] = newlines | ((followed || closed_by_end_of_data) ? kExtraResult : 0u) | (last_byte == '\n' ? kEndsOnNewline : 0u);
-    }
+    my_newlines = newlines;
+    }
+    return my_newlines;
 }
 
 __device__ __forceinline__ void settle_shared_word(unsigned long long *slot, uint32_t *word, uint32_t mine) {
@@ -156,7 +159,8 @@
 __device__ __forceinline__ void dfa2_body(const Dfa2Device &prog, const uint8_t *__restrict__ bytes, size_t nbytes, uint32_t stripe,
                                           const uint64_t *__restrict__ stripe_base, uint32_t *__restrict__ accept_bits,
                                           uint32_t *__restrict__ counts, uint32_t *__restrict__ slabs, PhaseHook phase = PhaseHook(),
-                                          uint32_t flush_mask = 31u, unsigned long long *__restrict__ slots = nullptr, uint64_t nwords = 0) {
+                                          uint32_t flush_mask = 31u, unsigned long long *__restrict__ slots = nullptr, uint64_t nwords = 0,
+                                          uint32_t *__restrict__ totals = nullptr) {
     static_assert(!OWN_WORDS || (!ONEPASS && KB == 1), "the exchange slots serve the indexed kernels with one bit per line");
     phase(kPhaseEntry);
     __shared__ __attribute__((aligned(16))) struct {
@@ -176,8 +180,10 @@
     const size_t g0 = (size_t)blockIdx.x * kThreads;
     uint64_t window_word = 0;
     if (!ONEPASS) window_word = (line_of(stripe_base[g0]) * KB) >> 5;
-    dfa2_stripe<ONEPASS, PhaseHook, FLUSH_SLOTS, KB, CLEAN, Dfa2T<PAIRS8>>(eng, g0 + threadIdx.x, window_word, stage, stage_words, bytes, nbytes, stripe, stripe_base, accept_bits,
-                                                            counts, slabs, gridDim.x * kThreads, phase, flush_mask);
+    const uint32_t wave = workgroup_wave();
+    const uint32_t my_newlines = dfa2_stripe<ONEPASS, PhaseHook, FLUSH_SLOTS, KB, CLEAN, Dfa2T<PAIRS8>>(
+        eng, g0 + threadIdx.x, window_word, stage, stage_words, bytes, nbytes, stripe, stripe_base, accept_bits, counts, slabs, gridDim.x * kThreads, phase, flush_mask);
+    if constexpr (ONEPASS) store_workgroup_total(my_newlines, wave, stage, totals);
     if constexpr (OWN_WORDS) {
         __syncthreads();
         const bool last = blockIdx.x + 1 == gridDim.x;
@@ -219,31 +225,35 @@
                                                                            uint32_t *__restrict__ wide_bits) {
     dfa2_body<false, 32, NoPhaseHook, 2>(prog, bytes, nbytes, stripe, stripe_base, wide_bits, nullptr, nullptr);
 }
+template <bool PAIRS8>
 __global__ __launch_bounds__(kThreads) void match_stripes2_onepass_kernel(Dfa2Device prog, const uint8_t *__restrict__ bytes, size_t nbytes,
                                                                            uint32_t stripe, uint32_t *__restrict__ counts,
-                                                                           uint32_t *__restrict__ slabs) {
-    dfa2_body<true, 32>(prog, bytes, nbytes, stripe, nullptr, nullptr, counts, slabs);
-}
-
-constexpr uint32_t kCompactWindowWords = 8192;
-__global__ __launch_bounds__(256) void compact_streams_kernel(const uint32_t *__restrict__ counts, const uint64_t *__restrict__ stripe_base,
-                                                               size_t nstripes, uint32_t stripe, const uint32_t *__restrict__ slabs,
-                                                               uint32_t *__restrict__ accept_bits, size_t cap_words) {
-    __shared__ uint32_t window[kCompactWindowWords];
-    const size_t g0 = (size_t)blockIdx.x * 256;
-    const size_t g1 = g0 + 256 < nstripes ? g0 + 256 : nstripes;
-    const uint64_t window_word = line_of(stripe_base[g0]) >> 5;
-    const uint64_t span = (line_of(stripe_base[g1]) >> 5) - window_word + 2;
+                                                                           uint32_t *__restrict__ slabs, uint32_t *__restrict__ totals) {
+    dfa2_body<true, 32, NoPhaseHook, 1, true, false, PAIRS8>(prog, bytes, nbytes, stripe, nullptr, nullptr, counts, slabs, NoPhaseHook(), 31u, nullptr, 0, totals);
+}
+
+constexpr uint32_t kCompactWindowWords = 32 * kThreads;
+__global__ __launch_bounds__(kThreads) void compact_streams_kernel(const uint32_t *__restrict__ counts, const uint32_t *__restrict__ totals,
+                                                                    size_t nstripes, uint32_t stripe, const uint32_t *__restrict__ slabs,
+                                                                    uint32_t *__restrict__ accept_bits, size_t cap_words,
+                                                                    const uint8_t *__restrict__ last_byte, uint64_t *__restrict__ mail) {
+    extern __shared__ uint32_t window[];
+    __shared__ uint64_t wave_tot[2][kThreads / 64];
+    const size_t g = (size_t)blockIdx.x * kThreads + threadIdx.x;
+    uint64_t part = 0;
+    for (uint32_t i = threadIdx.x; i < blockIdx.x; i += kThreads) part += totals[i];
+    uint64_t front, mine;
+    (void)block_exclusive_scan<kThreads / 64>(part, wave_tot[0], front);
+    const uint32_t c = g < nstripes ? counts[g] : 0u;
+    const uint64_t base = front + block_exclusive_scan<kThreads / 64>(c & kCountMask, wave_tot[1], mine);
+    const uint64_t window_word = front >> 5;
+    const uint64_t span = ((front + mine) >> 5) - window_word + 2;
     const uint32_t used = span < kCompactWindowWords ? (uint32_t)span : kCompactWindowWords;
-    for (uint32_t i = threadIdx.x; i < used; i += 256) window[i] = 0;
+    for (uint32_t i = threadIdx.x; i < used; i += kThreads) window[i] = 0;
     __syncthreads();
-    const size_t g = g0 + threadIdx.x;
     if (g < nstripes) {
-        const uint32_t c = counts[g];
         const uint32_t n = (c & kCountMask) + ((c & kExtraResult) ? 1u : 0u);
-        const uint64_t b = stripe_base[g];
-        const uint64_t base = line_of(b);
-        const bool fresh = (b & kFreshStripe) != 0;
+        const bool fresh = g == 0 || (counts[g - 1] & kEndsOnNewline) != 0;
         const size_t row = (nstripes + kThreads - 1) / kThreads * kThreads;
         const uint32_t *src = slabs + g;
         auto put = [&](uint64_t word, uint32_t v) {
@@ -264,9 +274,17 @@
         }
     }
     __syncthreads();
-    for (uint32_t i = threadIdx.x; i < used; i += 256) {
+    for (uint32_t i = threadIdx.x; i < used; i += kThreads) {
         const uint32_t v = window[i];
         if (v && window_word + i < cap_words) atomicOr(&accept_bits[window_word + i], v);
+    }
+    if (blockIdx.x + 1 == gridDim.x && threadIdx.x == 0) {
+        mail[0] = front + mine;
+        mail[1] = 0;
+        mail[2] = *last_byte;
+        mail[3] = 0;
+        mail[4] = 0;
+        __threadfence_system();
     }
 }
 
@@ -387,23 +405,29 @@
     return (int)hipGetLastError();
 }
 int match_onepass_dfa(const LineDfaDevice &p, const uint8_t *bytes, size_t nbytes, uint32_t stripe, size_t nstripes, uint32_t *counts,
-                      uint32_t *slabs, void *stream) {
-    if (p.in_global) return launch_onepass<LineDfaGlobalEngine, LineDfaDevice>(p, 256, bytes, nbytes, stripe, nstripes, counts, slabs, stream);
-    if (p.wide) return launch_onepass<LineDfaEngine<true, true>, LineDfaDevice>(p, LineDfaEngine<true, true>::lds_bytes(p), bytes, nbytes, stripe, nstripes, counts, slabs, stream);
-    return launch_onepass<LineDfaEngine<false, false>, LineDfaDevice>(p, LineDfaEngine<false, false>::lds_bytes(p), bytes, nbytes, stripe, nstripes, counts, slabs, stream);
+                      uint32_t *slabs, uint32_t *totals, void *stream) {
+    if (p.in_global) return launch_onepass<LineDfaGlobalEngine, LineDfaDevice>(p, 256, bytes, nbytes, stripe, nstripes, counts, slabs, totals, stream);
+    if (p.wide) return launch_onepass<LineDfaEngine<true, true>, LineDfaDevice>(p, LineDfaEngine<true, true>::lds_bytes(p), bytes, nbytes, stripe, nstripes, counts, slabs, totals, stream);
+    return launch_onepass<LineDfaEngine<false, false>, LineDfaDevice>(p, LineDfaEngine<false, false>::lds_bytes(p), bytes, nbytes, stripe, nstripes, counts, slabs, totals, stream);
 }
 size_t onepass_slab_words(size_t nstripes, uint32_t stripe) {
     return ((nstripes + kThreads - 1) / kThreads) * slab_words_per_lane(stripe) * kThreads;
 }
+size_t onepass_total_words(size_t nstripes) { return (nstripes + kThreads - 1) / kThreads; }
 int match_onepass_dfa2(const Dfa2Device &p, const uint8_t *bytes, size_t nbytes, uint32_t stripe, size_t nstripes, uint32_t *counts,
-                       uint32_t *slabs, void *stream) {
-    return launch_dfa2(match_stripes2_onepass_kernel, p, bytes, nbytes, stripe, nstripes, kThreads, stream, counts, slabs);
-}
-int compact_streams(const uint32_t *counts, const uint64_t *stripe_base, size_t nstripes, uint32_t stripe, const uint32_t *slabs,
-                    uint32_t *accept_bits, size_t cap_words, void *stream) {
+                       uint32_t *slabs, uint32_t *totals, void *stream) {
+    return p.P8 ? launch_dfa2(match_stripes2_onepass_kernel<true>, p, bytes, nbytes, stripe, nstripes, kThreads, stream, counts, slabs, totals)
+                : launch_dfa2(match_stripes2_onepass_kernel<false>, p, bytes, nbytes, stripe, nstripes, kThreads, stream, counts, slabs, totals);
+}
+int compact_streams(const uint32_t *counts, const uint32_t *totals, size_t nstripes, uint32_t stripe, const uint32_t *slabs,
+                    uint32_t *accept_bits, size_t cap_words, const uint8_t *last_byte, uint64_t *mail, void *stream) {
     if (!nstripes) return 0;
-    hipLaunchKernelGGL(compact_streams_kernel, dim3((unsigned)((nstripes + 255) / 256)), dim3(256), 0, (hipStream_t)stream, counts, stripe_base, nstripes,
-                       stripe, slabs, accept_bits, cap_words);
+    static LdsAttr attr;
+    const size_t lds = kCompactWindowWords * sizeof(uint32_t);
+    hipError_t e = ensure_dynamic_lds(attr, reinterpret_cast<const void *>(compact_streams_kernel), lds);
+    if (e != hipSuccess) return (int)e;
+    hipLaunchKernelGGL(compact_streams_kernel, dim3((unsigned)onepass_total_words(nstripes)), dim3(kThreads), lds, (hipStream_t)stream, counts, totals,
+                       nstripes, stripe, slabs, accept_bits, cap_words, last_byte, mail);
     return (int)hipGetLastError();
 }
 int match_extents_dfa(const DfaDevice &p, const uint8_t *bytes, const uint64_t *off, size_t nitems, uint32_t trim, uint8_t *accept,
```

Result: no change. 5666, median of 4 (+0.2%).
